# medical-genomics-group/VAMPomi

Hardware: AMD Instinct MI355X
Metric: VAMP iterations/s (+ achieved HBM GB/s of the A/A^T kernels) (higher is better)
Workload: dtype f64

## Files before the change

include/vampomi.h:

```cpp
#ifndef VAMPOMI_H
#define VAMPOMI_H

#include <stdint.h>

#ifdef __cplusplus
extern "C" {
#endif

#define VAMPOMI_ABI_VERSION 3
#define VAMPOMI_MAX_L 64
#define VAMPOMI_UNIQUE_ID_BYTES 128

typedef enum {
    VAMPOMI_OK = 0,
    VAMPOMI_ERR_ARG = 1,
    VAMPOMI_ERR_HIP = 2,
    VAMPOMI_ERR_RCCL = 3,
    VAMPOMI_ERR_IO = 4,
    VAMPOMI_ERR_NAN_PHEN = 5,
    VAMPOMI_ERR_STATE = 6,
    VAMPOMI_ERR_OOM = 7,
    VAMPOMI_ERR_MODEL = 8
} vampomi_status;

// ... 95 lines not shown
    int64_t a_passes_ref;
    int64_t a_passes_exec;
    double* prior_hist;
} vampomi_result;

void vampomi_params_default(vampomi_params* p);
vampomi_status vampomi_infere(vampomi_ctx* ctx, const vampomi_params* p, vampomi_result* r);
vampomi_status vampomi_vamp_begin(vampomi_ctx* ctx, const vampomi_params* p, vampomi_result* r);
vampomi_status vampomi_vamp_step(vampomi_ctx* ctx, int* stopped);
vampomi_status vampomi_vamp_end(vampomi_ctx* ctx);
vampomi_status vampomi_step_phases(vampomi_ctx* ctx, double* solve_s, double* step_s);

vampomi_status vampomi_assoc_loo(vampomi_ctx* ctx, const double* est, double* pvals, double* stats,
                                 int mem);
vampomi_status vampomi_assoc_se(vampomi_ctx* ctx, const double* r1, double gam1, double* pvals, int mem);

vampomi_status vampomi_test_metrics(vampomi_ctx* ctx, const double* est, double* r2, double* corr2, int mem);

typedef struct {
    int64_t launches;
    double ms_total;
    double bytes_total;
    double flops_total;
    int64_t timed;
    double ms_timed;
} vampomi_kernel_stat;

typedef struct {
    vampomi_kernel_stat ax;
    vampomi_kernel_stat atx;
    vampomi_kernel_stat ax_k[4];
    vampomi_kernel_stat atx_k[4];
    int64_t a_passes_exec;
    int64_t host_syncs;
    vampomi_kernel_stat loo;
    vampomi_kernel_stat op;
    vampomi_kernel_stat op_k[4];
    vampomi_kernel_stat coll;
} vampomi_stats;

vampomi_status vampomi_set_timing(vampomi_ctx* ctx, int on);
vampomi_status vampomi_get_stats(vampomi_ctx* ctx, vampomi_stats* out);
vampomi_status vampomi_reset_stats(vampomi_ctx* ctx);

vampomi_status vampomi_dev_set_variant(vampomi_ctx* ctx, int which, int variant);
vampomi_status vampomi_dev_prestep_counts(const vampomi_ctx* ctx, int64_t* made, int64_t* used);
vampomi_status vampomi_dev_time_pass(vampomi_ctx* ctx, int which, int K, int reps, double* avg_ms);
vampomi_status vampomi_dev_read_ceiling(vampomi_ctx* ctx, int reps, double* us_med, double* bytes, int* variant);
vampomi_status vampomi_dev_kernel_name(const vampomi_ctx* ctx, int which, int K, int mode, char* out, int cap);
vampomi_status vampomi_dev_ax_plan(int64_t N, int64_t M, int cus, int variant, int K, int* T, int* TR, int* S,
                                   int* grid, int* nslots, char* name, int cap);
vampomi_status vampomi_dev_op_plan(int64_t N, int64_t M, int cus, int variant, int K, int* T, int* S, int* TR,
                                   int* grid, int64_t* nslots, char* name, int cap);
vampomi_status vampomi_dev_op_lds(int64_t N, int64_t M, int cus, int variant, int K, int64_t* out);
vampomi_status vampomi_dev_op_timestamps(vampomi_ctx* ctx, unsigned long long* out, int cap, int* n);
vampomi_status vampomi_dev_mem_plan(int64_t N, int64_t Mt, int nranks, int rank, int cus, int probit, int writer,
                                    int64_t* bytes);
vampomi_status vampomi_dev_op_apply(vampomi_ctx* ctx, int K, const double* ar, const double* qo, const double* p,
                                    const double* z, const double* beta, double diag, double tau, double gam2,
                                    double* d, double* ad, double* dp);

#ifdef __cplusplus
}
#endif
#endif
```

vampomi_amd/_lib.py:

```python
from __future__ import annotations

import ctypes as C
import os

try:
    import torch
except Exception:
    torch = None

HERE = os.path.dirname(os.path.abspath(__file__))
LIB_PATH = os.environ.get("VAMPOMI_LIB") or os.path.join(HERE, "lib", "libvampomi.so")
CLI_PATH = os.path.join(HERE, "bin", "main_meth.exe")

MAX_L = 64
UNIQUE_ID_BYTES = 128
MEM_HOST, MEM_DEVICE = 0, 1
GEN_GAUSS, GEN_METH = 0, 1

STATUS = {
    0: "OK", 1: "ERR_ARG", 2: "ERR_HIP", 3: "ERR_RCCL", 4: "ERR_IO",
    5: "ERR_NAN_PHEN", 6: "ERR_STATE", 7: "ERR_OOM", 8: "ERR_MODEL",
}


# ... 60 lines not shown
    "vampomi_last_error": (C.c_char_p, []),
    "vampomi_divide_work": (None, [C.c_int64, C.c_int, C.c_int, C.POINTER(C.c_int64), C.POINTER(C.c_int64),
                                   C.POINTER(C.c_int64)]),
    "vampomi_comm_unique_id": (C.c_int, [_P]),
    "vampomi_open": (C.c_int, [C.POINTER(ShardDesc), C.POINTER(_P)]),
    "vampomi_close": (None, [_P]),
    "vampomi_shard_info": (C.c_int, [_P, C.POINTER(C.c_int64), C.POINTER(C.c_int64), C.POINTER(C.c_int64)]),
    "vampomi_sync": (C.c_int, [_P]),
    "vampomi_barrier": (C.c_int, [_P]),
    "vampomi_barrier_timeout": (C.c_int, [_P, C.c_double]),
    "vampomi_load_meth_file": (C.c_int, [_P, C.c_char_p]),
    "vampomi_load_meth_host": (C.c_int, [_P, _P, C.c_int64]),
    "vampomi_generate_meth": (C.c_int, [_P, C.c_uint64, C.c_int]),
    "vampomi_read_phen": (C.c_int, [_P, C.c_char_p, C.c_int]),
    "vampomi_set_phen": (C.c_int, [_P, _P, C.c_int]),
    "vampomi_get_phen": (C.c_int, [_P, _P]),
    "vampomi_simulate_phen": (C.c_int, [_P, C.c_uint64, C.c_double, C.c_double, _P]),
    "vampomi_simulate_phen_binary": (C.c_int, [_P, C.c_uint64, C.c_double, C.c_double, _P]),
    "vampomi_get_marker_stats": (C.c_int, [_P, _P, _P]),
    "vampomi_read_markers": (C.c_int, [_P, C.c_int64, C.c_int64, _P]),
    "vampomi_ax": (C.c_int, [_P, _P, _P, C.c_int]),
    "vampomi_atx": (C.c_int, [_P, _P, _P, C.c_int]),
    "vampomi_lmmse_mult": (C.c_int, [_P, _P, C.c_double, C.c_double, _P, C.c_int]),
    "vampomi_pcg": (C.c_int, [_P, _P, _P, C.c_double, C.c_double, C.c_int, C.c_int, C.c_double, _P,
                              C.POINTER(C.c_int), C.c_int]),
    "vampomi_test_metrics": (C.c_int, [_P, _P, C.POINTER(C.c_double), C.POINTER(C.c_double), C.c_int]),
    "vampomi_assoc_loo": (C.c_int, [_P, _P, _P, _P, C.c_int]),
    "vampomi_assoc_se": (C.c_int, [_P, _P, C.c_double, _P, C.c_int]),
    "vampomi_update_prior": (C.c_int, [_P, _P, C.c_double, C.POINTER(C.c_int), _P, _P, C.c_int, C.c_double,
                                        C.c_int, C.c_double, C.c_int]),
    "vampomi_denoise_bin": (C.c_int, [_P, _P, C.c_double, _P, C.POINTER(C.c_double), C.c_int]),
    "vampomi_denoise": (C.c_int, [_P, _P, C.c_double, _P, _P, C.c_int, _P, _P, C.POINTER(C.c_double), C.c_int]),
    "vampomi_params_default": (None, [C.POINTER(Params)]),
    "vampomi_infere": (C.c_int, [_P, C.POINTER(Params), C.POINTER(Result)]),
    "vampomi_vamp_begin": (C.c_int, [_P, C.POINTER(Params), C.POINTER(Result)]),
    "vampomi_vamp_step": (C.c_int, [_P, C.POINTER(C.c_int)]),
    "vampomi_step_phases": (C.c_int, [_P, C.POINTER(C.c_double), C.POINTER(C.c_double)]),
    "vampomi_vamp_end": (C.c_int, [_P]),
    "vampomi_set_timing": (C.c_int, [_P, C.c_int]),
    "vampomi_get_stats": (C.c_int, [_P, C.POINTER(Stats)]),
    "vampomi_reset_stats": (C.c_int, [_P]),
    "vampomi_dev_set_variant": (C.c_int, [_P, C.c_int, C.c_int]),
    "vampomi_dev_prestep_counts": (C.c_int, [_P, C.POINTER(C.c_int64), C.POINTER(C.c_int64)]),
    "vampomi_dev_time_pass": (C.c_int, [_P, C.c_int, C.c_int, C.c_int, C.POINTER(C.c_double)]),
    "vampomi_dev_read_ceiling": (C.c_int, [_P, C.c_int, C.POINTER(C.c_double), C.POINTER(C.c_double),
                                           C.POINTER(C.c_int)]),
    "vampomi_dev_kernel_name": (C.c_int, [_P, C.c_int, C.c_int, C.c_int, C.c_char_p, C.c_int]),
    "vampomi_dev_mem_plan": (C.c_int, [C.c_int64, C.c_int64, C.c_int, C.c_int, C.c_int, C.c_int, C.c_int, _P]),
    "vampomi_dev_ax_plan": (C.c_int, [C.c_int64, C.c_int64, C.c_int, C.c_int, C.c_int, _P, _P, _P, _P, _P, C.c_char_p,
                                      C.c_int]),
    "vampomi_dev_op_plan": (C.c_int, [C.c_int64, C.c_int64, C.c_int, C.c_int, C.c_int, _P, _P, _P, _P, _P, C.c_char_p,
                                      C.c_int]),
    "vampomi_dev_op_lds": (C.c_int, [C.c_int64, C.c_int64, C.c_int, C.c_int, C.c_int, _P]),
    "vampomi_dev_op_apply": (C.c_int, [_P, C.c_int, _P, _P, _P, _P, _P, C.c_double, C.c_double, C.c_double, _P, _P,
                                       _P]),
    "vampomi_dev_op_timestamps": (C.c_int, [_P, _P, C.c_int, C.POINTER(C.c_int)]),
    "vampomi_all_ok": (C.c_int, [_P, C.c_int, C.POINTER(C.c_int)]),
    "vampomi_comm_abort": (C.c_int, [_P]),
}

_lib = None


def load() -> C.CDLL:
    global _lib
    if _lib is None:
        if not os.path.exists(LIB_PATH):
            raise ImportError(f"{LIB_PATH} not built: run `python -m vampomi_amd.build`")
        lib = C.CDLL(LIB_PATH, mode=C.RTLD_GLOBAL)
        other = bool(os.environ.get("VAMPOMI_LIB"))
        for name, (res, args) in SIGNATURES.items():
            if other and not hasattr(lib, name):
                continue
            f = getattr(lib, name)
            f.restype = res
            f.argtypes = args
        _lib = lib
    return _lib


def check(status: int) -> None:
    if status != 0:
        msg = load().vampomi_last_error()
        raise VampomiError(status, msg.decode() if msg else "")
```

vampomi_amd/csrc/atax_team.hip:

```cpp
#include <hip/hip_ext.h>

#include <algorithm>
#include <cstdio>
#include <mutex>
#include <string>

#include "kdev.h"

namespace vk {

typedef unsigned int v4u __attribute__((ext_vector_type(4)));
typedef unsigned int v2u __attribute__((ext_vector_type(2)));

#ifndef TM_FMA
#define TM_FMA 1
#endif
#ifndef TM_SAFE
#define TM_SAFE 0
#endif
#ifndef TM_TS
#define TM_TS 0
#endif
#ifndef TM_TEAMS_BY_XCD
#define TM_TEAMS_BY_XCD 1
// ... 145 lines not shown
    const double* p[K];
    double* d[K];
    double* sraw[K];
    double diag[K], tau[K], gam2[K];
};
template <int K>
__device__ __forceinline__ TmSlots<K> tm_slots(const OpArgs& a, int alt) {
    TmSlots<K> s;
#pragma unroll
    for (int k = 0; k < K; ++k) {
        int idx = k == alt ? kOpMaxK : k;
        asm volatile("" : "+s"(idx));
        const OpAlt::Slot& t = a.alt.tab[idx];
        s.ar[k] = t.ar;
        s.p[k] = t.p;
        s.d[k] = t.d;
        s.sraw[k] = t.sraw;
        s.diag[k] = t.diag;
        s.tau[k] = t.tau;
        s.gam2[k] = t.gam2;
    }
    return s;
}

template <int K, int S, int F, int L, int P, bool COMM, int E, bool FMA, int KP>
__device__ __forceinline__ void atax_team_body(const double* __restrict__ X, int64_t ld, int64_t N, int64_t M,
                                               const double* __restrict__ mave, const double* __restrict__ msig,
                                               const OpArgs& a, int T, int TR, int ilv,
                                               const int* __restrict__ gate) {
    extern __shared__ __attribute__((aligned(16))) double lds[];
    double* s_beta = lds;
    if (a.fold.on) {
        double& s_go = lds[kOpMaxK];
        if (threadIdx.x == 0) {
            CgState cs = *a.fold.src;
            double r[3 * kMaxRhs];
#pragma unroll
            for (int q = 0; q < 3 * kMaxRhs; ++q) r[q] = q < 3 * cs.K ? a.fold.red[q] : 0.0;
            const bool ran = cg_decide_into(cs, r, a.fold.it, a.fold.mask);
            if (blockIdx.x == 0) {
                *a.fold.dst = cs;
                cg_publish(cs, ran, a.fold.it, a.fold.mirror, a.fold.flag, a.fold.seq, a.fold.pack);
            }
            s_go = cs.any ? 1.0 : 0.0;
#pragma unroll
            for (int k = 0; k < kOpMaxK; ++k) s_beta[k] = cs.beta[k];
        }
        __syncthreads();
        if (s_go == 0.0) return;
    } else if (gate && !*gate) {
        return;
    }
    const double* beta = a.fold.on ? s_beta : a.beta;
    static_assert(K + KP <= kMaxRhs, "partial slots per team");
    int fuse = a.fuse, alt = -1;
    if constexpr (KP == 0) {
        if (a.alt.cs && !a.fold.on) alt = cg_pre_slot(a.alt.cs->active, K, *a.alt.done == a.alt.token);
        if (alt >= 0) fuse &= ~(1 << alt);
    }
#if TM_TS
    const unsigned long long ts0 = __builtin_amdgcn_s_memrealtime();
#endif
    const int dbg = TM_ABL ? TM_ABL : (TM_DBG || !COMM) ? a.dbg : 0;
    constexpr int CW = COMM ? 7 : 8;
    constexpr int RS = tm_rows_per_step(COMM, E);
    static_assert(E == 1 || E == 2, "doubles per lane per load");
    constexpr int RING = F + L + 1;
    static_assert(COMM || L == 0, "without a hand-off the column is finished in its own step");
    static_assert(!COMM || (P >= 1 && P <= L), "polls in flight");
    static_assert(!COMM || P < RING, "a poll's slot is consumed before it is reissued");
    const int wave = threadIdx.x >> 6, lane = threadIdx.x & 63;
    const int g = blockIdx.x >> 3;
    const int member = g % T;
    const int nteams = gridDim.x / T;
#if TM_TEAMS_BY_XCD
    const int team = g / T + (nteams >> 3) * (int)(blockIdx.x & 7);
#else
    const int team = (blockIdx.x & 7) + 8 * (g / T);
#endif
    const int64_t cs = ilv ? nteams : 1;
    const int64_t mb = ilv ? team : (int64_t)team * M / nteams;
    const int n = (int)(ilv ? (M - team + nteams - 1) / nteams : (int64_t)(team + 1) * M / nteams - mb);
    const int64_t nmax = (M + nteams - 1) / nteams;
    const int64_t gwords = (M + gridDim.x) * kOpMaxK * T * 2;
    const int64_t r0 = (int64_t)member * TR;
    const int nrows = (int)(N - r0 < TR ? N - r0 : TR);
    constexpr bool QFULL = tm_qfull(K, S, COMM, E);
    const TmLds lay = tm_lds(K, S, COMM, E, TR < N ? TR : N);
    const int QS = (int)lay.qs;
    double* q_lds = lds + lay.q;
    double* s_part = lds + lay.part;
    double* s_tot = lds + lay.tot;
    const int jb = 64 * E * wave + E * lane;
    const int nbytes = (E == 2 ? (nrows + 1) & ~1 : nrows) * 8;

    if (COMM && wave == CW) {
        const TmSlots<K> sl = tm_slots<K>(a, alt);
        const int nq = K * T;
        unsigned long long* xg = a.xg + (int64_t)team * nmax * nq * 2;
        unsigned long long* dummy = a.xg + gwords + (int64_t)blockIdx.x * 2 * K;
        const bool qv = (lane >> 5) < K && (lane & 31) < T;
        const int ql2 = qv ? 2 * ((lane >> 5) * T + (lane & 31)) : 0;
        const int nq2 = 2 * nq;
        const int csi = (int)cs;
        const unsigned tag = a.tag;
        const double* scp = msig;
#pragma unroll
        for (int k = 0; k < K; ++k) {
            if (lane == 1 + k) scp = sl.p[k];
            if (lane == 1 + K + k && ((fuse >> k) & 1)) scp = a.z.p[k];
        }
// ... 301 lines not shown
                    if (threadIdx.x == 0) {
                        if (a.sraw.p[0]) sl.sraw[k][mg] = t;
                        sl.d[k][mg] = val;
                    }
                    dpacc[k] += val * p;
                }
                cc[k] = sg * val;
            }
        }
#pragma unroll
        for (int s = 0; s < S; ++s) {
            if (dbg & 8) break;
#pragma unroll
            for (int k = 0; k < K; ++k)
#pragma unroll
                for (int e = 0; e < E; ++e) {
                    if constexpr (FMA)
                        acc[k][s][e] = __builtin_fma(xr[slot][s][e], cc[k], acc[k][s][e]);
                    else
                        acc[k][s][e] += xr[slot][s][e] * cc[k];
                }
        }
    };
    if (n > 0) {
        for (int base = -F;; base += RING) {
            if (base - L >= n) break;
#pragma unroll
            for (int i = 0; i < RING; ++i) {
                const int m = base + i;
                load((i + F) % RING, m + F < n ? m + F : n - 1);
                if (m >= 0 && m < n) dot(i, m & 1);
                __syncthreads();
                const int cf = m - L;
                if (cf >= 0 && cf < n) {
                    double tot[K];
                    if (COMM) {
#pragma unroll
                        for (int k = 0; k < K; ++k) tot[k] = s_tot[(cf & 1) * K + k];
                    } else {
#pragma unroll
                        for (int k = 0; k < K; ++k) {
                            double t = 0.0;
#pragma unroll
                            for (int w = 0; w < CW; ++w) t += s_part[((m & 1) * CW + w) * K + k];
                            tot[k] = t;
                        }
                    }
                    finish((i + RING - L) % RING, cf, tot);
                }
            }
        }
    }
    double* dst = a.part + (int64_t)team * kMaxRhs * ld + r0;
#pragma unroll
    for (int s = 0; s < S; ++s) {
        const int jl = RS * s + jb;
        if (jl >= nrows) continue;
#pragma unroll
        for (int k = 0; k < K; ++k)
#pragma unroll
            for (int e = 0; e < E; ++e)
                if (jl + e < nrows) dst[(int64_t)k * ld + jl + e] = acc[k][s][e];
        if constexpr (KP > 0) {
#pragma unroll
            for (int k = 0; k < KP; ++k)
#pragma unroll
                for (int e = 0; e < E; ++e)
                    if (jl + e < nrows) dst[(int64_t)(K + k) * ld + jl + e] = accp[k][s][e];
        }
    }
    if constexpr (COMM) {
        __syncthreads();
    } else if (threadIdx.x == 0) {
#pragma unroll
        for (int k = 0; k < K; ++k) red_put(a.ro, (int64_t)blockIdx.x * K + k, dpacc[k]);
    }
    if (wave == 0) ticket_sum_blocks<K>(a.ro);
#if TM_TS
    if (a.ts && threadIdx.x == 0) {
        unsigned xcc, hw;
        asm volatile("s_getreg_b32 %0, hwreg(HW_REG_XCC_ID)" : "=s"(xcc));
        asm volatile("s_getreg_b32 %0, hwreg(HW_REG_HW_ID)" : "=s"(hw));
        unsigned long long* t = a.ts + 4 * (int64_t)blockIdx.x;
        t[0] = ts0;
        t[1] = __builtin_amdgcn_s_memrealtime();
        t[2] = xcc;
        t[3] = hw;
    }
#endif
}

template <int K, int S, int F, int L, int P, bool COMM, int E, bool FMA>
__global__ __launch_bounds__(kTmThreads) void atax_team_kernel(const double* __restrict__ X, int64_t ld, int64_t N,
                                                               int64_t M, const double* __restrict__ mave,
                                                               const double* __restrict__ msig, OpArgs a, int T,
                                                               int TR, int ilv, const int* __restrict__ gate) {
    atax_team_body<K, S, F, L, P, COMM, E, FMA, 0>(X, ld, N, M, mave, msig, a, T, TR, ilv, gate);
}

static constexpr int kTmPlain = kOpPlain;
template <int S, int F, int L, int P, bool COMM, int E, bool FMA>
__global__ __launch_bounds__(kTmThreads) void atax_team_plain_kernel(const double* __restrict__ X, int64_t ld,
                                                                     int64_t N, int64_t M,
                                                                     const double* __restrict__ mave,
                                                                     const double* __restrict__ msig, OpArgs a, int T,
                                                                     int TR, int ilv, const int* __restrict__ gate) {
    atax_team_body<1, S, F, L, P, COMM, E, FMA, kTmPlain>(X, ld, N, M, mave, msig, a, T, TR, ilv, gate);
}

#ifndef AX_TEAM_SYNC
#define AX_TEAM_SYNC 1
#endif
#ifndef AX_TEAM_F
#define AX_TEAM_F 4
#endif
static constexpr int kAxTmF = AX_TEAM_F;
static constexpr int kAxTmMaxS = 4;
template <int S, int KP, bool FU>
__global__ __launch_bounds__(kTmThreads) void ax_team_kernel(const double* __restrict__ X, int64_t ld, int64_t N,
                                                             int64_t M, const double* __restrict__ mave,
                                                             const double* __restrict__ msig, CPtrs xs,
                                                             double* __restrict__ part, AxFuse fu, int T, int TR) {
    if (fu.gate && !*fu.gate) return;
    constexpr int E = 2, F = kAxTmF, RING = F + 1;
    constexpr int RS = tm_rows_per_step(false, E);
    const int wave = threadIdx.x >> 6, lane = threadIdx.x & 63;
    const int g = blockIdx.x >> 3;
    const int member = g % T;
    const int nteams = gridDim.x / T;
    const int team = g / T + (nteams >> 3) * (int)(blockIdx.x & 7);
    const int n = team < M ? (int)((M - team + nteams - 1) / nteams) : 0;
    const int64_t r0 = (int64_t)member * TR;
    const int nrows = (int)(N - r0 < TR ? N - r0 : TR);
    const int nbytes = ((nrows + 1) & ~1) * 8;
    const int jb = 64 * E * wave + E * lane;
    double bk[KP];
#pragma unroll
    for (int k = 0; k < KP; ++k) bk[k] = FU ? fu.beta[k] : 0.0;
    const double* pkp = mave;
    if (lane == 1) pkp = msig;
#pragma unroll
    for (int k = 0; k < KP; ++k) {
        if (lane == 2 + k) pkp = xs.p[k];
        if (FU && lane == 2 + KP + k) pkp = fu.z.p[k];
    }
    pkp += team;
    double acc[KP][S][E];
#pragma unroll
    for (int k = 0; k < KP; ++k)
#pragma unroll
        for (int s = 0; s < S; ++s)
#pragma unroll
            for (int e = 0; e < E; ++e) acc[k][s][e] = 0.0;
    double xr[RING][S][E];
    double pk[RING];
    const char* xtile = reinterpret_cast<const char*>(X + (int64_t)team * ld + r0);
    auto load = [&](int slot, int m) {
        const int64_t c = (int64_t)m * nteams;
        pk[slot] = pkp[c];
        const __amdgpu_buffer_rsrc_t rs =
// ... 52 lines not shown
    }
}

static int tm_S(int64_t rows, bool comm, int E) {
    const int rs = tm_rows_per_step(comm, E);
    return (int)((rows + rs - 1) / rs);
}

bool team_plan(int64_t N, int64_t M, int cus, int T, int cfg, OpPlan* out) {
    if (cfg < 0 || cfg >= kTmNCfg || N < 1) return false;
    const TmCfg& c = kTmCfg[cfg];
    if ((T == 1) == c.comm) return false;
    if (T < 1 || T > kTmMaxT || (T & (T - 1))) return false;
    const int grid = (cus / (8 * T)) * 8 * T;
    if (grid < T) return false;
    int64_t TR = N;
    if (T > 1) {
        TR = c.E == 2 ? ((N + T - 1) / T + 127) / 128 * 128 : (N + T - 1) / T;
        if ((int64_t)(T - 1) * TR >= N) return false;
    }
    const int S = tm_S(TR, c.comm, c.E);
    if (S > c.maxS) return false;
    for (int K = 1; K <= kOpMaxK; ++K)
        if (tm_lds(K, S, c.comm, c.E, std::min<int64_t>(TR, N)).words * 8 > kTmLdsMaxBytes) return false;
    OpPlan p{};
    p.grid = grid;
    p.S = S;
    p.T = T;
    p.TR = (int)TR;
    p.cfg = cfg;
    p.nslots = grid / T;
    (void)M;
    *out = p;
    return true;
}

bool team_lds_layout(const OpPlan& pl, int64_t N, int K, int64_t out[6]) {
    if (pl.T < 1 || pl.cfg < 0 || pl.cfg >= kTmNCfg || K < 1 || K > kOpMaxK || N < 1) return false;
    const TmCfg& c = kTmCfg[pl.cfg];
    const TmLds l = tm_lds(K, pl.S, c.comm, c.E, std::min<int64_t>(pl.TR, N));
    out[0] = kTmLdsHead;
    out[1] = l.q;
    out[2] = l.qs;
    out[3] = l.part;
    out[4] = l.tot;
    out[5] = l.words;
    return true;
}

template <int K, int S, int C, bool PL>
static hipError_t launch_tm(const Shard& s, const OpPlan& pl, const OpArgs& a, hipStream_t st, const Timing& tm,
                            const int* gate, int* occ) {
    constexpr TmCfg c = kTmCfg[C];
    static_assert(!PL || K == 1, "the head-start kernel has one operator system");
    void (*kern)(const double*, int64_t, int64_t, int64_t, const double*, const double*, OpArgs, int, int, int,
                 const int*);
    if constexpr (PL)
        kern = atax_team_plain_kernel<S, c.F, c.L, c.P, c.comm, c.E, (bool)TM_FMA>;
    else
        kern = atax_team_kernel<K, S, c.F, c.L, c.P, c.comm, c.E, (bool)TM_FMA>;
    const size_t lds = (size_t)tm_lds(K, S, c.comm, c.E, std::min<int64_t>(pl.TR, s.N)).words * sizeof(double);
    if (lds > (size_t)kTmLdsMaxBytes) return hipErrorInvalidValue;
    static std::atomic<unsigned long long> allowed{0};
    if (const hipError_t e = lds_allow(reinterpret_cast<const void*>(kern), allowed, (int)kTmLdsMaxBytes))
        return e;
    if (occ) {
        if (hipOccupancyMaxActiveBlocksPerMultiprocessor(occ, kern, kTmThreads, lds) != hipSuccess) *occ = 0;
        return hipSuccess;
    }
    hipExtLaunchKernelGGL(kern, dim3(pl.grid), dim3(kTmThreads), lds, st, tm.start, tm.stop, 0, s.X, s.ld, s.N, s.M,
                          s.mave, s.msig, a, pl.T, pl.TR, c.ilv ? 1 : 0, gate);
    return hipSuccess;
}

static constexpr int tm_plain_maxS(int cfg) {
    return cfg == 0 ? 8 : cfg == 2 ? 3 : cfg == 3 ? 4 : cfg == 4 ? 5 : 0;
}

template <int K, int C, int S, bool PL>
static hipError_t launch_tm_if(const Shard& s, const OpPlan& pl, const OpArgs& a, hipStream_t st, const Timing& tm,
                               const int* gate, int* occ) {
    if constexpr (S <= (PL ? tm_plain_maxS(C) : kTmCfg[C].maxS))
        return launch_tm<K, S, C, PL>(s, pl, a, st, tm, gate, occ);
    return hipErrorInvalidValue;
}

template <int K, int C, bool PL>
static hipError_t launch_tm_s(int S, const Shard& s, const OpPlan& pl, const OpArgs& a, hipStream_t st,
                        const Timing& tm, const int* gate, int* occ) {
    switch (S) {
        case 1: return launch_tm_if<K, C, 1, PL>(s, pl, a, st, tm, gate, occ);
        case 2: return launch_tm_if<K, C, 2, PL>(s, pl, a, st, tm, gate, occ);
        case 3: return launch_tm_if<K, C, 3, PL>(s, pl, a, st, tm, gate, occ);
        case 4: return launch_tm_if<K, C, 4, PL>(s, pl, a, st, tm, gate, occ);
        case 5: return launch_tm_if<K, C, 5, PL>(s, pl, a, st, tm, gate, occ);
        case 6: return launch_tm_if<K, C, 6, PL>(s, pl, a, st, tm, gate, occ);
        case 7: return launch_tm_if<K, C, 7, PL>(s, pl, a, st, tm, gate, occ);
        case 8: return launch_tm_if<K, C, 8, PL>(s, pl, a, st, tm, gate, occ);
        case 9: return launch_tm_if<K, C, 9, PL>(s, pl, a, st, tm, gate, occ);
        case 10: return launch_tm_if<K, C, 10, PL>(s, pl, a, st, tm, gate, occ);
        default: return hipErrorInvalidValue;
    }
}

static OpArgs tm_with_slots(const OpArgs& a, int K) {
    OpArgs x = a;
    for (int k = 0; k < K && k < kOpMaxK; ++k)
        x.alt.tab[k] = OpAlt::Slot{a.ar.p[k], a.p.p[k], a.d.p[k], a.sraw.p[k], a.diag, a.tau, a.gam2};
    x.alt.tab[kOpMaxK] = OpAlt::Slot{a.alt.ar, a.alt.p, a.alt.d, a.sraw.p[0] ? a.alt.d : nullptr, 1.0, 1.0, 0.0};
    return x;
}

template <int K, bool PL = false>
static hipError_t launch_tm_c(const Shard& s, const OpPlan& pl, const OpArgs& a0, hipStream_t st, const Timing& tm,
                        const int* gate, int* occ = nullptr) {
    const OpArgs a = tm_with_slots(a0, K);
    if constexpr (PL) {
        switch (pl.cfg) {
            case 0: return launch_tm_s<1, 0, true>(pl.S, s, pl, a, st, tm, gate, occ);
            case 2: return launch_tm_s<1, 2, true>(pl.S, s, pl, a, st, tm, gate, occ);
            case 3: return launch_tm_s<1, 3, true>(pl.S, s, pl, a, st, tm, gate, occ);
            case 4: return launch_tm_s<1, 4, true>(pl.S, s, pl, a, st, tm, gate, occ);
            default: return hipErrorInvalidValue;
        }
    }
    switch (pl.cfg) {
        case 0: return launch_tm_s<K, 0, false>(pl.S, s, pl, a, st, tm, gate, occ);
        case 1: return launch_tm_s<K, 1, false>(pl.S, s, pl, a, st, tm, gate, occ);
        case 2: return launch_tm_s<K, 2, false>(pl.S, s, pl, a, st, tm, gate, occ);
        case 3: return launch_tm_s<K, 3, false>(pl.S, s, pl, a, st, tm, gate, occ);
        case 4: return launch_tm_s<K, 4, false>(pl.S, s, pl, a, st, tm, gate, occ);
        case 5: return launch_tm_s<K, 5, false>(pl.S, s, pl, a, st, tm, gate, occ);
        case 6: return launch_tm_s<K, 6, false>(pl.S, s, pl, a, st, tm, gate, occ);
        default: return hipErrorInvalidValue;
    }
}

hipError_t atax_team(const Shard& s, const OpPlan& pl, int K, const OpArgs& a, hipStream_t st, const Timing& tm,
                     const int* gate) {
    if (pl.T < 1 || pl.grid < pl.T || pl.grid % pl.T) return hipErrorInvalidValue;
    if (pl.T > 1 && (!a.xg || !a.err || a.tag == 0)) return hipErrorInvalidValue;
    if (s.M <= 0) return hipSuccess;
    hipError_t e = hipErrorInvalidValue;
    switch (K) {
        case 1: e = launch_tm_c<1>(s, pl, a, st, tm, gate); break;
        case 2: e = launch_tm_c<2>(s, pl, a, st, tm, gate); break;
        default: break;
    }
    if (e != hipSuccess) return e;
    return hipGetLastError();
}

hipError_t atax_team_plain(const Shard& s, const OpPlan& pl, const OpArgs& a, hipStream_t st, const Timing& tm,
                           const int* gate) {
    if (pl.T < 1 || pl.grid < pl.T || pl.grid % pl.T) return hipErrorInvalidValue;
    if (pl.T > 1 && (!a.xg || !a.err || a.tag == 0)) return hipErrorInvalidValue;
    for (int k = 0; k < kTmPlain; ++k)
        if (!a.px.p[k]) return hipErrorInvalidValue;
    if (s.M <= 0) return hipSuccess;
    if (const hipError_t e = launch_tm_c<1, true>(s, pl, a, st, tm, gate)) return e;
    return hipGetLastError();
}

bool ax_team_plan(int64_t N, int64_t M, int cus, AxPlan* out) {
    if (N < 1 || cus < 8) return false;
    constexpr int RS = tm_rows_per_step(false, 2);
    for (int T = 1; T <= kTmMaxT; T *= 2) {
        if (cus / (8 * T) < 1) break;
        const int grid = (cus / (8 * T)) * 8 * T;
        const int64_t TR = T == 1 ? N : ((N + T - 1) / T + 127) / 128 * 128;
        if ((int64_t)(T - 1) * TR >= N) continue;
        const int S = (int)((TR + RS - 1) / RS);
        if (S > kAxTmMaxS) continue;
        AxPlan p{};
        p.variant = kAxTeam;
        p.T = T;
        p.TR = (int)TR;
        p.S = S;
        p.groups = grid;
        p.nslots = grid / T;
        p.rows = N;
        p.tiles = 1;
        p.total = M;
        p.sa = p.nslots;
        p.sb = 1;
        *out = p;
        return true;
    }
    return false;
}

template <int S, int K, bool FU>
static void launch_axt(const Shard& s, const AxPlan& pl, CPtrs x, double* part, hipStream_t st, const Timing& tm,
                       const AxFuse& fu) {
    hipExtLaunchKernelGGL((ax_team_kernel<S, K, FU>), dim3(pl.groups), dim3(kTmThreads), 0, st, tm.start, tm.stop, 0,
                          s.X, s.ld, s.N, s.M, s.mave, s.msig, x, part, fu, pl.T, pl.TR);
}

template <int S>
static bool launch_axt_k(int K, bool fused, const Shard& s, const AxPlan& pl, CPtrs x, double* part,
                         hipStream_t st, const Timing& tm, const AxFuse& fu) {
    switch (K * 2 + (fused ? 1 : 0)) {
        case 2: launch_axt<S, 1, false>(s, pl, x, part, st, tm, fu); return true;
        case 3: launch_axt<S, 1, true>(s, pl, x, part, st, tm, fu); return true;
        case 4: launch_axt<S, 2, false>(s, pl, x, part, st, tm, fu); return true;
        case 5: launch_axt<S, 2, true>(s, pl, x, part, st, tm, fu); return true;
        case 6: launch_axt<S, 3, false>(s, pl, x, part, st, tm, fu); return true;
        case 7: launch_axt<S, 3, true>(s, pl, x, part, st, tm, fu); return true;
        case 8: launch_axt<S, 4, false>(s, pl, x, part, st, tm, fu); return true;
        case 9: launch_axt<S, 4, true>(s, pl, x, part, st, tm, fu); return true;
        default: return false;
    }
}

hipError_t ax_team(const Shard& s, const AxPlan& pl, int K, CPtrs x, double* part, hipStream_t st, const Timing& tm,
                   const AxFuse& fu) {
    if (pl.T < 1 || pl.groups % (8 * pl.T) || pl.nslots != pl.groups / pl.T || pl.S < 1 || pl.S > kAxTmMaxS ||
        (int64_t)(pl.T - 1) * pl.TR >= s.N || (int64_t)pl.T * pl.TR < s.N ||
        (int64_t)pl.S * tm_rows_per_step(false, 2) < std::min<int64_t>(pl.TR, s.N) || pl.rows < s.N)
        return hipErrorInvalidValue;
    if (s.M <= 0) return hipSuccess;
    const bool fused = fu.z.p[0] != nullptr;
    if (fused && !fu.beta) return hipErrorInvalidValue;
    bool ok = false;
    switch (pl.S) {
        case 1: ok = launch_axt_k<1>(K, fused, s, pl, x, part, st, tm, fu); break;
        case 2: ok = launch_axt_k<2>(K, fused, s, pl, x, part, st, tm, fu); break;
        case 3: ok = launch_axt_k<3>(K, fused, s, pl, x, part, st, tm, fu); break;
        case 4: ok = launch_axt_k<4>(K, fused, s, pl, x, part, st, tm, fu); break;
        default: break;
    }
    if (!ok) return hipErrorInvalidValue;
    return hipGetLastError();
}

std::string ax_kernel_name(int K, bool fused, const AxPlan& pl) {
    if (pl.T <= 0) return kernel_name(0, K, fused ? 1 : 0, pl.variant);
    char b[96];
    std::snprintf(b, sizeof b, "ax_team_kernel<%d, %d, %s>", pl.S, K, fused ? "true" : "false");
    return b;
}

bool team_plain_plan(int64_t N, int64_t M, int cus, const OpPlan& main, OpPlan* out) {
    const int cfgs1[] = {0};
    const int cfgsT[] = {2, 3, 4};
    for (int T = std::max(main.T, 1); T <= kTmMaxT; T *= 2) {
        const int* cf = T == 1 ? cfgs1 : cfgsT;
        const int ncf = T == 1 ? 1 : 3;
        for (int i = 0; i < ncf; ++i) {
            OpPlan p{};
            if (!team_plan(N, M, cus, T, cf[i], &p) || p.S > tm_plain_maxS(cf[i])) continue;
            *out = p;
            return true;
        }
    }
    return false;
}

int team_occupancy(const OpPlan& pl, int K) {
    int occ = 0;
    const Shard s{nullptr, 0, (int64_t)pl.TR * pl.T, 1, nullptr, nullptr};
    const OpArgs a{};
    hipError_t e = hipErrorInvalidValue;
    switch (K) {
        case 1: e = launch_tm_c<1>(s, pl, a, nullptr, Timing{}, nullptr, &occ); break;
        case 2: e = launch_tm_c<2>(s, pl, a, nullptr, Timing{}, nullptr, &occ); break;
        case 1 + kTmPlain: e = launch_tm_c<1, true>(s, pl, a, nullptr, Timing{}, nullptr, &occ); break;
        default: break;
    }
    return e == hipSuccess ? occ : 0;
}

std::string team_kernel_name(int K, const OpPlan& pl) {
    const TmCfg& c = kTmCfg[pl.cfg];
    char b[128];
    if (K == 1 + kTmPlain)
        std::snprintf(b, sizeof b, "atax_team_plain_kernel<%d, %d, %d, %d, %s, %d>", pl.S, c.F, c.L, c.P,
                      c.comm ? "true" : "false", c.E);
    else
        std::snprintf(b, sizeof b, "atax_team_kernel<%d, %d, %d, %d, %d, %s, %d>", K, pl.S, c.F, c.L, c.P,
                      c.comm ? "true" : "false", c.E);
    return b;
}

}
```

vampomi_amd/csrc/ctx.h:

```cpp
#pragma once
#include <hip/hip_runtime.h>
#include <rccl/rccl.h>

#include <cstdint>
#include <initializer_list>
#include <memory>
#include <string>
#include <utility>
#include <vector>

#include "../../include/vampomi.h"
#include "kernels.h"

vampomi_status fail(vampomi_status s, const std::string& msg);

#define HIPCHK(expr)                                                                                  \
    do {                                                                                              \
        hipError_t _e = (expr);                                                                       \
        if (_e != hipSuccess)                                                                         \
            return fail(VAMPOMI_ERR_HIP, std::string(#expr) + ": " + hipGetErrorString(_e));          \
    } while (0)

#define NCCLCHK(expr)                                                                                 \
    do {                                                                                              \
// ... 44 lines not shown
    bool mr_tail_req = true;
    bool cg_fold = true;
    bool dp_separate = false;
    bool team_reg = false;
    hipEvent_t team_ev = nullptr;
    ncclComm_t comm = nullptr;
    bool use_comm = false;
    std::shared_ptr<LoopbackComm> loopback;
    std::shared_ptr<ShmComm> shm;
    uint64_t coll_seq = 0;
    bool aborted = false;

    double* X = nullptr;
    double* mave = nullptr;
    double* msig = nullptr;
    double* y = nullptr;
    std::vector<double> y_host;
    bool have_X = false, have_y = false;

    vk::AxPlan axp{};
    int atx_variant = vk::kAtxDefault, loo_variant = vk::kLooDefault;
    double* ax_part = nullptr;
    double* red_part = nullptr;
    size_t red_cap = 0;
    double* scal = nullptr;
    double* h_scal = nullptr;
    double* d_hscal = nullptr;
    unsigned* ticket = nullptr;
    unsigned long long* h_flag = nullptr;
    unsigned long long* d_flag = nullptr;
    unsigned long long sync_seq = 0;
    vk::CgState* cgs = nullptr;
    vk::CgMirror* h_cgm = nullptr;
    vk::CgMirror* d_cgm = nullptr;
    vk::OpPlan opp{};
    int op_variant = vk::kOpDefault;
    bool op_ready = false;
    bool op_ok_mine = false;
    bool op_ok = false;
    bool op_agreed = false;
    int op_variant_req = vk::kOpDefault;
    int cus = 0;
    double* op_part = nullptr;
    int64_t op_part_slots = 0;
    double* op_nvec = nullptr;
    unsigned long long* op_xg = nullptr;
    size_t op_xg_words = 0;
    unsigned op_tag = 0;
    vk::OpPlan opp_hs{};
    bool hs_ok_mine = false;
    bool hs_ok = false;
    bool hs_on = true;
    bool hs_on_req = true;
    int pre_mode = 2;
    unsigned long long pre_seq = 0;
    int64_t pre_made_n = 0, pre_used_n = 0;
    unsigned long long* op_ts = nullptr;
    double* nbuf = nullptr;
    double* mbuf = nullptr;

    bool timing = false;
    int tperiod = 1;
    int64_t tcount[5][vk::kMaxRhs] = {};
    std::vector<TimedLaunch> pending;
    std::vector<hipEvent_t> ev_pool;
    vampomi_stats stats{};

    std::unique_ptr<VampRun> run;
    std::unique_ptr<IterWriter> writer;

    vk::Shard shard() const { return vk::Shard{X, ld, N, M, mave, msig}; }
    vampomi_ctx();
    ~vampomi_ctx();
};

vampomi_status dev_alloc(double** p, size_t n);
void dev_free(double*& p);
vampomi_status host_sync(vampomi_ctx* c);
vampomi_status wait_flag(vampomi_ctx* c, unsigned long long seq, int word = 0);
vampomi_status sync_stream(vampomi_ctx* c, hipStream_t st);
vampomi_status allreduce_dev(vampomi_ctx* c, double* buf, size_t n, const char* site = __builtin_FUNCTION(),
                             int line = __builtin_LINE());
vampomi_status sum_over_ranks(vampomi_ctx* c, double local, double* total, const char* site = __builtin_FUNCTION(),
                              int line = __builtin_LINE());
void comm_abort(vampomi_ctx* c, const std::string& why);
void resolve_timing(vampomi_ctx* c);
TimedLaunch launch_stat(vampomi_ctx* c, int cls, int K, double bytes, double flops);
void drop_launches(vampomi_ctx* c, size_t pending_mark, const vampomi_stats& before);
void release_ctx_resources(vampomi_ctx* c);

vampomi_status ax_dev(vampomi_ctx* c, int K, const double* const* x, double* outbase,
                      const vk::AxFuse* fu = nullptr, const vk::DotArgs* tail = nullptr);
vampomi_status atx_dev(vampomi_ctx* c, int K, const double* const* u, double* const* out, int mode, double tau,
                       double gam2, const double* const* p, const int* gate = nullptr,
                       const double* const* zf = nullptr, const double* beta = nullptr, bool dp = true,
                       double* const* sraw = nullptr);
vampomi_status lmmse_dev(vampomi_ctx* c, int K, const double* const* v, double* const* d, double tau, double gam2,
                         double* nscratch);

class DotBatch {
   public:
    explicit DotBatch(vampomi_ctx* c) : c_(c) {}
    vampomi_status add(std::initializer_list<vk::DotTerm> terms, int64_t n, bool sync, double* out);
    struct Group {
        std::vector<vk::DotTerm> terms;
        bool sync;
// ... 5 lines not shown
    vampomi_status add_pair(int64_t na, const std::vector<Group>& ga, const vk::G1Chain* chain,
                            const double* chain_of, const std::vector<std::pair<const double*, double*>>& ca,
                            int64_t nb, const std::vector<Group>& gb,
                            const std::vector<std::pair<const double*, double*>>& cb);
    vampomi_status sink(int nq, bool sync, double* out, vk::RedOut* ro);
    vampomi_status flush();
    bool empty() const { return sinks_.empty(); }
    const double* dev_result(const double* out) const;
    vampomi_status reduce_now();
    double* dev_slot(const double* out) const;
    hipStream_t stream() const;

   private:
    vampomi_status build(const std::vector<Group>& groups, const vk::G1Chain* chain, const double* chain_of,
                         const std::vector<std::pair<const double*, double*>>& copies, vk::DotArgs& a,
                         vk::RedOut& ro);
    struct Sink {
        int slot, count;
        double* out;
    };
    vampomi_ctx* c_;
    int nsync_ = 0, nlocal_ = 0;
    int nred_ = 0;
    unsigned long long last_seq_ = 0;
    std::vector<Sink> sinks_;
};

inline vk::DotTerm T(const double* a, const double* b, int op = vk::DOT) { return vk::DotTerm{a, b, op}; }

struct CgSystem {
    const double* v = nullptr;
    double* mu = nullptr;
    bool mu0_nonzero = false;
    const double* atx0 = nullptr;
    double* W = nullptr;
    double* S = nullptr;
    double* AW = nullptr;
    bool onsager = false;
    int iters = 0;
    double *r = nullptr, *z = nullptr, *p = nullptr, *d = nullptr;
};
struct HeadStart {
    double* abern = nullptr;
    const double* xnext = nullptr;
    double* axnext = nullptr;
    bool used = false;
    double* T1 = nullptr;
    double* U1 = nullptr;
    unsigned long long* pre_done = nullptr;
    bool pre_have = false;
    bool pre_offer = false;
    bool pre_made = false;
    bool pre_used = false;
};
enum class PreMode { normal, ahead, queued };
struct PcgArgs {
    double tau = 0.0, gam2 = 0.0;
    int max_iter = 0;
    double tol = 0.0;
    double* nscratch = nullptr;
    int64_t* ref_passes = nullptr;
    DotBatch* init = nullptr;
    const double* extra_x = nullptr;
    double* ex_out = nullptr;
    bool onepass = false;
    const double* const* ar0 = nullptr;
    HeadStart* hs = nullptr;
    const vk::Prelude* pre = nullptr;
    PreMode pm = PreMode::normal;
};
vampomi_status pcg_run(vampomi_ctx* c, const std::vector<CgSystem*>& sys, const PcgArgs& args);
vampomi_status op_prepare(vampomi_ctx* c);
vampomi_status op_agree(vampomi_ctx* c);
vampomi_status headstart_available(vampomi_ctx* c, bool* yes);
constexpr int64_t kPreMinBytes = (int64_t)256 << 20;
bool prestep_on(const vampomi_ctx* c);
unsigned* op_err_dev(vampomi_ctx* c);
vampomi_status op_check_err(vampomi_ctx* c);
vampomi_status op_dev(vampomi_ctx* c, int K, const vk::OpArgs& a, const int* gate, bool reduce = true,
                      bool divide = true);
vampomi_status op_dev_plain(vampomi_ctx* c, const vk::OpArgs& a, const double* const* px, double* const* out,
                            const int* gate);
```

vampomi_amd/csrc/engine.cpp:

```cpp
#include <hip/hip_runtime.h>
#include <rccl/rccl.h>

#include <algorithm>
#include <atomic>
#include <cfloat>
#include <chrono>
#include <condition_variable>
#include <map>
#include <mutex>
#include <cmath>
#include <cstdio>
#include <cstdlib>
#include <cstring>
#include <memory>
#include <string>
#include <thread>
#include <vector>

#include <fcntl.h>
#include <unistd.h>

#include "ctx.h"
#include "hostio.h"
#include "writer.h"
// ... 605 lines not shown
        HIPCHK(vk::ax_reduce(c->axp, K, c->N, c->ld, c->ax_part, os, c->sqrtN, c->st, f.gate));
    } else {
        HIPCHK(vk::ax_reduce(c->axp, K, c->N, c->ld, c->ax_part, os, 0.0, c->st, f.gate));
        size_t n = (size_t)K * c->ld;
        if (tail) {
            HIPCHK(vk::dots(*tail, c->M, vk::RedOut{c->red_part, outbase + n, c->ticket, nullptr, 0, f.gate}, c->st));
            n += (size_t)tail->nt;
        }
        STCHK(allreduce_dev(c, outbase, n));
        HIPCHK(vk::vec_div(K, c->N, c->ld, os, c->sqrtN, c->st));
    }
    return VAMPOMI_OK;
}

vampomi_status atx_dev(vampomi_ctx* c, int K, const double* const* u, double* const* out, int mode,
                              double tau, double gam2, const double* const* p, const int* gate,
                              const double* const* zf, const double* beta, bool dp, double* const* sraw) {
    if (!c->have_X) return fail(VAMPOMI_ERR_STATE, "ATx before the methylation data was loaded");
    if (c->M <= 0) return VAMPOMI_OK;
    vk::CPtrs us{}, ps{}, zs{};
    vk::Ptrs os{}, ss{};
    for (int k = 0; k < K; ++k) {
        us.p[k] = u[k];
        os.p[k] = out[k];
        ss.p[k] = sraw ? sraw[k] : nullptr;
        ps.p[k] = p ? p[k] : nullptr;
        zs.p[k] = zf ? zf[k] : nullptr;
    }
    TimedLaunch t = launch_stat(c, 1, K, pass_bytes(c, K), pass_flops(c, K));
    HIPCHK(vk::atx(c->shard(), K, us, os, 1.0 / c->sqrtN, mode, tau, gam2, ps, c->st, c->atx_variant, vk::Timing{t.a, t.b}, gate, zs,
                   zf ? beta : nullptr, ss));
    c->stats.a_passes_exec++;
    if (mode == 1 && dp) {
        vk::DotArgs a{};
        a.nt = K;
        for (int k = 0; k < K; ++k)
            a.t[k] = zf ? vk::DotTerm{out[k], p[k], vk::PUPD, zf[k], beta + k} : vk::DotTerm{out[k], p[k], vk::DOT};
        HIPCHK(vk::dots(a, c->M, vk::RedOut{c->red_part, c->scal + SL_DP, c->ticket, nullptr, 0, gate}, c->st));
        STCHK(allreduce_dev(c, c->scal + SL_DP, K));
    }
    return VAMPOMI_OK;
}

static size_t red_capacity(int64_t Mx) {
    return std::max<size_t>({(size_t)vk::kRedBlocks * 3 * vk::kMaxRhs, (size_t)vk::kRedBlocks * vk::kMaxTerms,
                             (size_t)((Mx + 255) / 256) * (1 + 2 * (vk::kMaxL - 1)),
                             (size_t)(Mx / 8 + 1) * vk::kMaxRhs, (size_t)4096});
}

static size_t op_xg_words_for(int64_t Mx, const vk::OpPlan& p) {
    return (size_t)(Mx + p.grid) * vk::kOpMaxK * (size_t)p.T * 2 + (size_t)p.grid * (2 * vk::kOpMaxK + 1);
}

static vampomi_status op_plan_local(vampomi_ctx* c) {
    if (c->cus <= 0) HIPCHK(hipDeviceGetAttribute(&c->cus, hipDeviceAttributeMultiprocessorCount, c->device));
    const int64_t M = std::max<int64_t>(c->M, 1);
    bool op_ok = vk::op_plan(c->N, M, c->cus, c->op_variant, &c->opp);
    if (op_ok && c->opp.T >= 1) {
        for (int K = 1; K <= vk::kOpMaxK && op_ok; ++K) {
            const int occ = vk::team_occupancy(c->opp, K);
            if ((int64_t)occ * c->cus < c->opp.grid) {
                std::fprintf(stderr, "libvampomi: one-pass operator off: %s fits %d workgroup(s) per CU; the plan "
                                     "needs %lld resident on %d CUs (two passes per CG step)\n",
                             vk::team_kernel_name(K, c->opp).c_str(), occ, (long long)c->opp.grid, c->cus);
                op_ok = false;
            }
        }
    }
    bool hs_ok = op_ok && vk::team_plain_plan(c->N, M, c->cus, c->opp, &c->opp_hs);
    if (hs_ok && (int64_t)vk::team_occupancy(c->opp_hs, 1 + vk::kOpPlain) * c->cus < c->opp_hs.grid) hs_ok = false;
    c->op_ok_mine = op_ok;
    c->hs_ok_mine = hs_ok;
    if (!c->op_ts && std::getenv("VAMPOMI_OP_TS") && std::atoi(std::getenv("VAMPOMI_OP_TS"))) {
        HIPCHK(hipMalloc((void**)&c->op_ts, (size_t)4 * 8 * std::max(c->cus, 1) * 2));
        HIPCHK(hipMemsetAsync(c->op_ts, 0, (size_t)4 * 8 * std::max(c->cus, 1) * 2, c->st));
    }
    if (!c->op_nvec) {
        STCHK(dev_alloc(&c->op_nvec, (size_t)3 * vk::kMaxRhs * c->ld + 16));
        HIPCHK(hipMemsetAsync(c->op_nvec, 0, ((size_t)3 * vk::kMaxRhs * c->ld + 16) * 8, c->st));
    }
    if (op_ok) {
        const int64_t slots = std::max<int64_t>(c->opp.nslots, hs_ok ? c->opp_hs.nslots : 0);
        if (slots > c->op_part_slots) {
            dev_free(c->op_part);
            STCHK(dev_alloc(&c->op_part, (size_t)slots * vk::kMaxRhs * c->ld));
            c->op_part_slots = slots;
        }
        if (c->opp.T > 1 || (hs_ok && c->opp_hs.T > 1)) {
            size_t words = c->opp.T > 1 ? op_xg_words_for(M, c->opp) : 0;
            if (hs_ok && c->opp_hs.T > 1) words = std::max(words, op_xg_words_for(M, c->opp_hs));
            if (words > c->op_xg_words) {
                if (c->op_xg) (void)hipFree(c->op_xg);
                c->op_xg = nullptr;
                c->op_xg_words = 0;
                HIPCHK(hipMalloc((void**)&c->op_xg, words * 8));
                HIPCHK(hipMemsetAsync(c->op_xg, 0, words * 8, c->st));
                c->op_xg_words = words;
            }
        }
    }
    c->op_ready = true;
    return VAMPOMI_OK;
}

vampomi_status op_prepare(vampomi_ctx* c) {
    if (!c->op_ready) STCHK(op_plan_local(c));
    if (!c->use_comm) {
        c->op_ok = c->op_ok_mine;
        c->hs_ok = c->hs_ok_mine && c->hs_on;
    } else if (!c->op_agreed) {
        c->op_ok = c->hs_ok = false;
    }
    return VAMPOMI_OK;
}

vampomi_status op_agree(vampomi_ctx* c) {
    if (!c->use_comm) return VAMPOMI_OK;
    if (c->op_variant_req != c->op_variant || c->hs_on_req != c->hs_on) {
        c->op_variant = c->op_variant_req;
        c->hs_on = c->hs_on_req;
        c->op_ready = false;
    }
    bool op = false, hs = false;
    if (c->have_X) {
        if (!c->op_ready) STCHK(op_plan_local(c));
        op = c->op_ok_mine;
        hs = c->hs_ok_mine;
    }
    const double mine = (op ? 0.0 : 1.0) + (hs ? 0.0 : 1024.0) + (c->hs_on ? 0.0 : 1048576.0) +
                        (c->mr_tail_req ? 0.0 : 1073741824.0);
    double all = 0.0;
    STCHK(sum_over_ranks(c, mine, &all));
    const int64_t a = (int64_t)all;
    c->op_ok = a % 1024 == 0;
    c->hs_ok = c->op_ok && (a / 1024) % 1024 == 0 && (a / 1048576) % 1024 == 0;
    c->mr_tail = a / 1073741824 == 0;
    c->op_agreed = true;
    return VAMPOMI_OK;
// ... 63 lines not shown
    HIPCHK(launch());
    if (!g.last) HIPCHK(hipEventCreateWithFlags(&g.last, hipEventDisableTiming));
    HIPCHK(hipEventRecord(g.last, c->st));
    return VAMPOMI_OK;
}

vampomi_status op_check_err(vampomi_ctx* c) {
    const unsigned e = c->h_flag ? __atomic_exchange_n(reinterpret_cast<unsigned*>(c->h_flag + 4), 0u, __ATOMIC_ACQ_REL) : 0u;
    if (e > 1)
        return fail(VAMPOMI_ERR_HIP, "one-pass operator: address checks failed (codes " + std::to_string(e >> 1) + ")");
    if (e)
        return fail(VAMPOMI_ERR_HIP, "one-pass operator: a team hand-off timed out (a workgroup of the team never "
                                     "ran: fewer compute units than planned?)");
    return VAMPOMI_OK;
}

vampomi_status op_dev(vampomi_ctx* c, int K, const vk::OpArgs& a, const int* gate, bool reduce, bool divide) {
    if (!c->have_X) return fail(VAMPOMI_ERR_STATE, "A before the methylation data was loaded");
    STCHK(op_prepare(c));
    if (!c->op_ok || K < 1 || K > vk::kOpMaxK)
        return fail(VAMPOMI_ERR_ARG, "one-pass operator: K <= 2 and a plan for N = " + std::to_string(c->N));
    double* ad = c->op_nvec + (int64_t)2 * vk::kMaxRhs * c->ld;
    vk::OpArgs x = a;
    x.part = c->op_part;
    x.scale = 1.0 / c->sqrtN;
    if (c->opp.T > 1) {
        x.xg = c->op_xg;
        if (++c->op_tag == 0) ++c->op_tag;
        x.tag = c->op_tag;
        x.err = op_err_dev(c);
    }
    static const int dbg = std::getenv("VAMPOMI_OP_DBG") ? std::atoi(std::getenv("VAMPOMI_OP_DBG")) : 0;
    x.dbg = dbg;
    x.ts = c->op_ts;
    x.ro = vk::RedOut{c->red_part, c->use_comm ? ad + (int64_t)K * c->ld : c->scal + SL_DP, c->ticket, nullptr, 0,
                      gate};
    TimedLaunch t = launch_stat(c, 3, K, pass_bytes(c, K), 2.0 * pass_flops(c, K));
    STCHK(team_launch(c, c->opp.T,
                      [&] { return vk::atax(c->shard(), c->opp, K, x, c->st, vk::Timing{t.a, t.b}, gate); }));
    c->stats.a_passes_exec++;
    vk::Ptrs os{};
    for (int k = 0; k < K; ++k) os.p[k] = ad + (int64_t)k * c->ld;
    if (!c->use_comm) {
        if (reduce) HIPCHK(vk::op_reduce(c->opp, K, c->N, c->ld, c->op_part, os, c->sqrtN, c->st, gate));
    } else {
        HIPCHK(vk::op_reduce(c->opp, K, c->N, c->ld, c->op_part, os, 0.0, c->st, gate));
        STCHK(allreduce_dev(c, ad, (size_t)K * c->ld + K));
        if (divide) HIPCHK(vk::vec_div(K, c->N, c->ld, os, c->sqrtN, c->st));
    }
    return VAMPOMI_OK;
}

vampomi_status op_dev_plain(vampomi_ctx* c, const vk::OpArgs& a, const double* const* px, double* const* out,
                            const int* gate) {
    if (!c->have_X) return fail(VAMPOMI_ERR_STATE, "A before the methylation data was loaded");
    STCHK(op_prepare(c));
    if (!c->hs_ok) return fail(VAMPOMI_ERR_ARG, "head-start launch: no plan for N = " + std::to_string(c->N));
    constexpr int KT = 1 + vk::kOpPlain;
    double* ad = c->op_nvec + (int64_t)2 * vk::kMaxRhs * c->ld;
    vk::OpArgs x = a;
    x.part = c->op_part;
    x.scale = 1.0 / c->sqrtN;
    for (int k = 0; k < vk::kOpPlain; ++k) x.px.p[k] = px[k];
    if (c->opp_hs.T > 1) {
        x.xg = c->op_xg;
        if (++c->op_tag == 0) ++c->op_tag;
        x.tag = c->op_tag;
        x.err = op_err_dev(c);
    }
    x.dbg = 0;
    x.ro = vk::RedOut{c->red_part, c->use_comm ? ad + (int64_t)KT * c->ld : c->scal + SL_DP, c->ticket, nullptr, 0,
                      gate};
    TimedLaunch t = launch_stat(c, 3, KT, pass_bytes(c, KT), pass_flops(c, 1) + pass_flops(c, KT));
    STCHK(team_launch(c, c->opp_hs.T, [&] {
        return vk::atax_team_plain(c->shard(), c->opp_hs, x, c->st, vk::Timing{t.a, t.b}, gate);
    }));
    c->stats.a_passes_exec++;
    if (!c->use_comm) {
        vk::Ptrs os{};
        for (int k = 0; k < vk::kOpPlain; ++k) os.p[k] = out[k];
        HIPCHK(vk::op_reduce(c->opp_hs, vk::kOpPlain, c->N, c->ld, c->op_part, os, c->sqrtN, c->st, gate, 1));
    } else {
        vk::Ptrs os{};
        for (int k = 0; k < KT; ++k) os.p[k] = ad + (int64_t)k * c->ld;
        HIPCHK(vk::op_reduce(c->opp_hs, KT, c->N, c->ld, c->op_part, os, 0.0, c->st, gate));
        STCHK(allreduce_dev(c, ad, (size_t)KT * c->ld + 1));
        vk::Ptrs dst = os;
        for (int k = 0; k < vk::kOpPlain; ++k) dst.p[1 + k] = out[k];
        HIPCHK(vk::vec_div(KT, c->N, c->ld, os, c->sqrtN, c->st, &dst));
    }
    return VAMPOMI_OK;
}

vampomi_status lmmse_dev(vampomi_ctx* c, int K, const double* const* v, double* const* d, double tau,
                                double gam2, double* nscratch) {
    STCHK(ax_dev(c, K, v, nscratch));
    const double* u[vk::kMaxRhs];
    for (int k = 0; k < K; ++k) u[k] = nscratch + (int64_t)k * c->ld;
    return atx_dev(c, K, u, d, 1, tau, gam2, v);
}

extern "C" int vampomi_abi_version(void) { return VAMPOMI_ABI_VERSION; }
extern "C" const char* vampomi_last_error(void) { return g_err.c_str(); }

extern "C" void vampomi_divide_work(int64_t Mt, int nranks, int rank, int64_t* M, int64_t* S, int64_t* Mm) {
    const int64_t modu = Mt % nranks, size = Mt / nranks;
    int64_t cum = 0;
    for (int r = 0; r < nranks; ++r) {
        const int64_t len = r < modu ? size + 1 : size;
        if (r == rank) {
            if (M) *M = len;
            if (S) *S = cum;
        }
        cum += len;
    }
    if (Mm) *Mm = modu != 0 ? size + 1 : size;
}

extern "C" vampomi_status vampomi_comm_unique_id(void* out) {
    if (!out) return fail(VAMPOMI_ERR_ARG, "null argument");
    ncclUniqueId id;
    NCCLCHK(ncclGetUniqueId(&id));
    static_assert(sizeof(ncclUniqueId) == VAMPOMI_UNIQUE_ID_BYTES, "unique id size");
    std::memcpy(out, &id, sizeof id);
    return VAMPOMI_OK;
}

void release_ctx_resources(vampomi_ctx* c) {
    (void)hipSetDevice(c->device);
    if (c->st) (void)hipStreamSynchronize(c->st);
    team_gate_leave(c);
    resolve_timing(c);
    for (auto e : c->ev_pool) (void)hipEventDestroy(e);
    c->ev_pool.clear();
// ... 41 lines not shown
    if (d->Mt < d->nranks) return fail(VAMPOMI_ERR_ARG, "every rank needs at least one marker (Mt >= nranks)");
    std::unique_ptr<vampomi_ctx> c(new vampomi_ctx());
    c->rank = d->rank;
    c->nranks = d->nranks;
    c->N = d->N;
    c->Mt = d->Mt;
    c->alpha_scale = d->alpha_scale == 0.0 ? 1.0 : d->alpha_scale;
    vampomi_divide_work(c->Mt, c->nranks, c->rank, &c->M, &c->S, &c->Mm);
    c->ld = (c->N + 15) / 16 * 16;
    c->sqrtN = std::sqrt((double)c->N);
    int ndev = 0;
    HIPCHK(hipGetDeviceCount(&ndev));
    if (ndev < 1) return fail(VAMPOMI_ERR_HIP, "no HIP device visible");
    c->device = d->device >= 0 ? d->device : c->rank % ndev;
    HIPCHK(hipSetDevice(c->device));
    HIPCHK(hipStreamCreateWithFlags(&c->st, hipStreamNonBlocking));
    team_gate_join(c.get());
    const int64_t Mx = std::max<int64_t>(c->M, 1);
    c->axp = vk::ax_plan(c->N, Mx);
    STCHK(dev_alloc(&c->mave, Mx));
    STCHK(dev_alloc(&c->msig, Mx));
    STCHK(dev_alloc(&c->y, c->ld));
    HIPCHK(hipMemsetAsync(c->y, 0, c->ld * 8, c->st));
    STCHK(dev_alloc(&c->ax_part, (size_t)c->axp.nslots * vk::kMaxRhs * c->ld));
    c->red_cap = red_capacity(Mx);
    STCHK(dev_alloc(&c->red_part, c->red_cap));
    c->writer.reset(new IterWriter());
    STCHK(c->writer->open(c.get()));
    STCHK(dev_alloc(&c->scal, SL_TOTAL));
    HIPCHK(hipHostMalloc((void**)&c->h_scal, SL_TOTAL * sizeof(double), hipHostMallocMapped | hipHostMallocCoherent));
    HIPCHK(hipHostGetDevicePointer((void**)&c->d_hscal, c->h_scal, 0));
    HIPCHK(hipHostMalloc((void**)&c->h_flag, 64, hipHostMallocMapped | hipHostMallocCoherent));
    std::memset(c->h_flag, 0, 64);
    HIPCHK(hipHostGetDevicePointer((void**)&c->d_flag, c->h_flag, 0));
    HIPCHK(hipMalloc((void**)&c->ticket, 64 * sizeof(unsigned)));
    HIPCHK(hipMemsetAsync(c->ticket, 0, 64 * sizeof(unsigned), c->st));
    STCHK(dev_alloc(&c->nbuf, (size_t)vk::kMaxRhs * c->ld));
    HIPCHK(hipMemsetAsync(c->nbuf, 0, (size_t)vk::kMaxRhs * c->ld * 8, c->st));
    STCHK(dev_alloc(&c->mbuf, (size_t)2 * vk::kMaxRhs * Mx));
    HIPCHK(hipMalloc((void**)&c->cgs, 2 * sizeof(vk::CgState)));
    HIPCHK(hipMemsetAsync(c->cgs, 0, 2 * sizeof(vk::CgState), c->st));
    HIPCHK(hipHostMalloc((void**)&c->h_cgm, vk::kCgMirrorSlots * sizeof(vk::CgMirror),
                         hipHostMallocMapped | hipHostMallocCoherent));
    std::memset(c->h_cgm, 0, vk::kCgMirrorSlots * sizeof(vk::CgMirror));
    HIPCHK(hipHostGetDevicePointer((void**)&c->d_cgm, c->h_cgm, 0));
    const char* force = std::getenv("VAMPOMI_FORCE_RCCL");
    c->use_comm = c->nranks > 1 || (force && std::atoi(force) != 0);
    if (const char* mv = std::getenv("VAMPOMI_MR_TAIL")) c->mr_tail = c->mr_tail_req = std::atoi(mv) != 0;
    if (const char* fv = std::getenv("VAMPOMI_CG_FOLD")) c->cg_fold = std::atoi(fv) != 0;
    if (const char* dv = std::getenv("VAMPOMI_DP_SEPARATE")) c->dp_separate = std::atoi(dv) != 0;
    if (const char* hv = std::getenv("VAMPOMI_HEADSTART")) c->hs_on = c->hs_on_req = std::atoi(hv) != 0;
    if (const char* pv = std::getenv("VAMPOMI_PRESTEP")) {
        const int v = std::atoi(pv);
        if (v >= 0 && v <= 2) c->pre_mode = v;
    }
    const char* mode = std::getenv("VAMPOMI_COMM");
    if (c->use_comm && mode && std::strcmp(mode, "loopback") == 0) {
        if (!d->comm_id) return fail(VAMPOMI_ERR_ARG, "the loopback communicator needs a communicator id");
        c->loopback = loopback_join(d->comm_id, c->nranks);
    } else if (c->use_comm && mode && std::strcmp(mode, "shm") == 0) {
        if (!d->comm_id) return fail(VAMPOMI_ERR_ARG, "the shm communicator needs a communicator id");
        std::string err;
        c->shm = shm_join(d->comm_id, c->nranks, c->rank, comm_init_timeout_s(), &err);
        if (!c->shm) return fail(VAMPOMI_ERR_STATE, err);
    } else if (c->use_comm) {
        ncclUniqueId id;
        if (d->comm_id)
            std::memcpy(&id, d->comm_id, sizeof id);
        else
            NCCLCHK(ncclGetUniqueId(&id));
        ncclConfig_t cfg = NCCL_CONFIG_INITIALIZER;
        cfg.blocking = 0;
        STCHK(nccl_settle(c.get(), ncclCommInitRankConfig(&c->comm, c->nranks, id, c->rank, &cfg),
                          "ncclCommInitRankConfig", comm_init_timeout_s()));
    }
    STCHK(sync_stream(c.get(), c->st));
    *out = c.release();
    return VAMPOMI_OK;
}

extern "C" vampomi_status vampomi_shard_info(const vampomi_ctx* c, int64_t* M, int64_t* S, int64_t* ld) {
    if (!c) return fail(VAMPOMI_ERR_ARG, "null context");
    if (M) *M = c->M;
    if (S) *S = c->S;
    if (ld) *ld = c->ld;
    return VAMPOMI_OK;
}

extern "C" vampomi_status vampomi_sync(vampomi_ctx* c) {
    if (!c) return fail(VAMPOMI_ERR_ARG, "null context");
    HIPCHK(hipSetDevice(c->device));
    STCHK(sync_stream(c, c->st));
    return VAMPOMI_OK;
}

extern "C" vampomi_status vampomi_barrier(vampomi_ctx* c) {
    CollScope cs_(c);
    if (!c) return fail(VAMPOMI_ERR_ARG, "null context");
    if (c->use_comm) STCHK(allreduce_dev(c, c->scal + SL_BARRIER, 1));
    STCHK(sync_stream(c, c->st));
    return VAMPOMI_OK;
}

extern "C" vampomi_status vampomi_barrier_timeout(vampomi_ctx* c, double seconds) {
    if (!c || !(seconds > 0)) return fail(VAMPOMI_ERR_ARG, "null context or no limit");
    c->coll_limit_s = seconds;
    const vampomi_status st = vampomi_barrier(c);
// ... 460 lines not shown
    for (auto pr : {std::make_pair(&out->ax, out->ax_k), std::make_pair(&out->atx, out->atx_k),
                    std::make_pair(&out->op, out->op_k)}) {
        int64_t n = 0;
        double ms = 0.0;
        for (int k = 0; k < 4; ++k) {
            n += pr.second[k].launches;
            ms += pr.second[k].ms_total;
        }
        if (n == pr.first->launches) pr.first->ms_total = ms;
        else fill(*pr.first);
    }
    return VAMPOMI_OK;
}

extern "C" vampomi_status vampomi_reset_stats(vampomi_ctx* c) {
    if (!c) return fail(VAMPOMI_ERR_ARG, "null context");
    STCHK(sync_stream(c, c->st));
    resolve_timing(c);
    c->stats = vampomi_stats{};
    return VAMPOMI_OK;
}

extern "C" vampomi_status vampomi_dev_set_variant(vampomi_ctx* c, int which, int variant) {
    if (!c) return fail(VAMPOMI_ERR_ARG, "null context");
    HIPCHK(hipSetDevice(c->device));
    STCHK(sync_stream(c, c->st));
    if (which == 0) {
        if (!vk::ax_variant_ok(variant)) return fail(VAMPOMI_ERR_ARG, "no such A.x variant");
        const vk::AxPlan np = vk::ax_plan(c->N, std::max<int64_t>(c->M, 1), variant);
        if (np.nslots > c->axp.nslots) {
            dev_free(c->ax_part);
            STCHK(dev_alloc(&c->ax_part, (size_t)np.nslots * vk::kMaxRhs * c->ld));
        }
        c->axp = np;
    } else if (which == 1) {
        if (!vk::atx_variant_ok(variant)) return fail(VAMPOMI_ERR_ARG, "no such A^T.u variant");
        c->atx_variant = variant;
    } else if (which == 3) {
        vk::OpPlan p{};
        if (!vk::op_plan(c->N, std::max<int64_t>(c->M, 1), c->cus > 0 ? c->cus : 256, variant, &p))
            return fail(VAMPOMI_ERR_ARG, "no such one-pass operator plan for this N");
        c->op_variant_req = variant;
        if (!c->use_comm) {
            c->op_variant = variant;
            c->op_ready = false;
        }
    } else if (which == 4) {
        return fail(VAMPOMI_ERR_ARG, "no side stream: every launch runs on the context's stream (DESIGN.md §6)");
    } else if (which == 5) {
        if (variant != 0 && variant != 1) return fail(VAMPOMI_ERR_ARG, "head start: 0 or 1");
        c->hs_on_req = variant == 1;
        if (!c->use_comm) c->hs_on = c->hs_on_req;
    } else if (which == 7) {
        if (variant < 0 || variant > 2) return fail(VAMPOMI_ERR_ARG, "pre-step: 0, 1 or 2");
        c->pre_mode = variant;
    } else if (which == 6) {
        if (variant != 0 && variant != 1) return fail(VAMPOMI_ERR_ARG, "multi-rank tail: 0 or 1");
        c->mr_tail_req = variant == 1;
        if (!c->use_comm) c->mr_tail = c->mr_tail_req;
    } else {
        if (!vk::loo_variant_ok(variant)) return fail(VAMPOMI_ERR_ARG, "no such association-pass variant");
        c->loo_variant = variant;
    }
    return VAMPOMI_OK;
}

bool prestep_on(const vampomi_ctx* c) {
    if (c->use_comm || c->nranks != 1 || !c->hs_ok || c->pre_mode == 0) return false;
    return c->pre_mode == 1 || std::max<int64_t>(c->M, 1) * c->ld * 8 >= kPreMinBytes;
}

extern "C" vampomi_status vampomi_dev_prestep_counts(const vampomi_ctx* c, int64_t* made, int64_t* used) {
    if (!c || !made || !used) return fail(VAMPOMI_ERR_ARG, "null argument");
    *made = c->pre_made_n;
    *used = c->pre_used_n;
    return VAMPOMI_OK;
}

extern "C" vampomi_status vampomi_dev_time_pass(vampomi_ctx* c, int which, int K, int reps, double* avg_ms) {
    if (!c || !avg_ms || K < 1 || K > (which == 0 ? 4 : which == 1 ? 3 : which == 3 ? 2 : 1) || reps < 1)
        return fail(VAMPOMI_ERR_ARG, "bad argument");
    if (!c->have_X) return fail(VAMPOMI_ERR_STATE, "no methylation data loaded");
    HIPCHK(hipSetDevice(c->device));
    if (which == 3) {
        STCHK(op_prepare(c));
        if (!c->op_ok_mine) return fail(VAMPOMI_ERR_ARG, "no one-pass operator plan for this N");
    }
    const int64_t Mx = std::max<int64_t>(c->M, 1);
    vk::CPtrs in{};
    vk::Ptrs out{};
    for (int k = 0; k < K; ++k) {
        in.p[k] = which == 0 ? c->mbuf + k * Mx : c->nbuf + k * c->ld;
        out.p[k] = which == 0 ? c->nbuf + k * c->ld : c->mbuf + k * Mx;
    }
    hipEvent_t a, b;
    HIPCHK(hipEventCreate(&a));
    HIPCHK(hipEventCreate(&b));
    HIPCHK(hipEventRecord(a, c->st));
    for (int r = 0; r < reps; ++r) {
        if (which == 0)
            HIPCHK(vk::ax_partial(c->shard(), c->axp, K, in, c->ax_part, c->st));
        else if (which == 1)
            HIPCHK(vk::atx(c->shard(), K, in, out, 1.0 / c->sqrtN, 0, 0.0, 0.0, vk::CPtrs{}, c->st, c->atx_variant));
        else if (which == 3) {
            vk::OpArgs x{};
            for (int k = 0; k < K; ++k) {
                x.ar.p[k] = c->nbuf + k * c->ld;
                x.p.p[k] = c->mbuf + k * Mx;
                x.d.p[k] = c->mbuf + (2 + k) * Mx;
            }
            x.diag = 1.0;
            x.scale = 1.0 / c->sqrtN;
            x.tau = 1.0;
            x.part = c->op_part;
            x.ro = vk::RedOut{c->red_part, c->scal + SL_DP, c->ticket, nullptr, 0, nullptr};
            if (c->opp.T > 1) {
                x.xg = c->op_xg;
                if (++c->op_tag == 0) ++c->op_tag;
                x.tag = c->op_tag;
                x.err = op_err_dev(c);
            }
            x.dbg = std::getenv("VAMPOMI_OP_DBG") ? std::atoi(std::getenv("VAMPOMI_OP_DBG")) : 0;
// ... 54 lines not shown
        a.fuse = (1 << K) - 1;
    }
    a.diag = diag;
    a.tau = tau;
    a.gam2 = gam2;
    STCHK(op_dev(c, K, a, nullptr));
    const double* AD = c->op_nvec + (int64_t)2 * vk::kMaxRhs * c->ld;
    for (int k = 0; k < K; ++k) {
        STCHK(stage_out(c, c->mbuf + (2 + k) * Mx, c->M, VAMPOMI_MEM_HOST, d + k * c->M));
        STCHK(stage_out(c, AD + k * c->ld, c->N, VAMPOMI_MEM_HOST, ad + k * c->N));
    }
    HIPCHK(hipMemcpyAsync(dp, c->scal + SL_DP, (size_t)K * 8, hipMemcpyDeviceToHost, c->st));
    STCHK(sync_stream(c, c->st));
    return op_check_err(c);
}

extern "C" vampomi_status vampomi_dev_op_timestamps(vampomi_ctx* c, unsigned long long* out, int cap, int* n) {
    if (!c || !out || !n) return fail(VAMPOMI_ERR_ARG, "null argument");
    if (!c->op_ts) return fail(VAMPOMI_ERR_STATE, "no timestamps (VAMPOMI_OP_TS=1 at the first operator use)");
    STCHK(sync_stream(c, c->st));
    *n = std::min(cap, 4 * c->opp.grid);
    HIPCHK(hipMemcpy(out, c->op_ts, (size_t)*n * 8, hipMemcpyDeviceToHost));
    return VAMPOMI_OK;
}

extern "C" vampomi_status vampomi_dev_ax_plan(int64_t N, int64_t M, int cus, int variant, int K, int* T, int* TR,
                                              int* S, int* grid, int* nslots, char* name, int cap) {
    if (N < 1 || M < 1 || cus < 1 || K < 1 || K > vk::kMaxRhs || !vk::ax_variant_ok(variant))
        return fail(VAMPOMI_ERR_ARG, "bad argument");
    const vk::AxPlan p = vk::ax_plan_for(N, M, cus, variant);
    if (T) *T = p.T;
    if (TR) *TR = p.TR;
    if (S) *S = p.S;
    if (grid) *grid = p.groups;
    if (nslots) *nslots = p.nslots;
    if (name && cap > 0) std::snprintf(name, (size_t)cap, "%s", vk::ax_kernel_name(K, false, p).c_str());
    return VAMPOMI_OK;
}

extern "C" vampomi_status vampomi_dev_op_plan(int64_t N, int64_t M, int cus, int variant, int K, int* T, int* S,
                                              int* TR, int* grid, int64_t* nslots, char* name, int cap) {
    vk::OpPlan p{};
    if (K < 1 || K > vk::kOpMaxK || !vk::op_plan(N, std::max<int64_t>(M, 1), cus, variant, &p))
        return fail(VAMPOMI_ERR_ARG, "no one-pass operator plan");
    if (T) *T = p.T;
    if (S) *S = p.S;
    if (TR) *TR = p.TR;
    if (grid) *grid = p.grid;
    if (nslots) *nslots = p.nslots;
    if (name && cap > 0) std::snprintf(name, (size_t)cap, "%s", vk::op_kernel_name(K, p).c_str());
    return VAMPOMI_OK;
}

extern "C" vampomi_status vampomi_dev_op_lds(int64_t N, int64_t M, int cus, int variant, int K, int64_t* out) {
    vk::OpPlan p{};
    if (!out || !vk::op_plan(N, std::max<int64_t>(M, 1), cus, variant, &p) || !vk::team_lds_layout(p, N, K, out))
        return fail(VAMPOMI_ERR_ARG, "no team plan with that system count");
    return VAMPOMI_OK;
}

extern "C" vampomi_status vampomi_dev_mem_plan(int64_t N, int64_t Mt, int nranks, int rank, int cus, int probit,
                                               int writer, int64_t* bytes) {
    if (!bytes || N < 2 || Mt < nranks || nranks < 1 || rank < 0 || rank >= nranks || cus < 1)
        return fail(VAMPOMI_ERR_ARG, "bad argument");
    int64_t M = 0, S = 0, Mm = 0;
    vampomi_divide_work(Mt, nranks, rank, &M, &S, &Mm);
    const int64_t Mx = std::max<int64_t>(M, 1), ld = (N + 15) / 16 * 16;
    int64_t total = 0;
    auto add = [&](int64_t n, int64_t elem) {
        const int64_t b = std::max<int64_t>(n, 1) * elem, g = 2 << 20;
        total += (b + g - 1) / g * g;
    };
    const vk::AxPlan axp = vk::ax_plan(N, Mx);
    add(Mx * ld, 8);
    add(Mx, 8), add(Mx, 8), add(ld, 8);
    add((int64_t)axp.nslots * vk::kMaxRhs * ld, 8);
    add((int64_t)red_capacity(Mx), 8), add((int64_t)red_capacity(Mx), 8);
    add(SL_TOTAL, 8), add(64, 4), add(64, 4);
    add((int64_t)vk::kMaxRhs * ld, 8);
    add((int64_t)2 * vk::kMaxRhs * Mx, 8);
    add((int64_t)sizeof(vk::CgState), 1);
    vk::OpPlan op{}, hs{};
    if (vk::op_plan(N, Mx, cus, vk::kOpDefault, &op)) {
        const bool h = vk::team_plain_plan(N, Mx, cus, op, &hs);
        add((int64_t)3 * vk::kMaxRhs * ld + 16, 8);
        add(std::max<int64_t>(op.nslots, h ? hs.nslots : 0) * vk::kMaxRhs * ld, 8);
        size_t w = op.T > 1 ? op_xg_words_for(Mx, op) : 0;
        if (h && hs.T > 1) w = std::max(w, op_xg_words_for(Mx, hs));
        if (w) add((int64_t)w, 8);
    }
    for (int q = 0; q < 25; ++q) add(Mx, 8);
    add(ld, 8), add((int64_t)vk::kMaxRhs * ld, 8), add((int64_t)vk::kMaxRhs * ld, 8), add(ld, 8);
    add(2 * ld, 8);
    add(Mx, 8), add(ld + 2, 8);
    if (probit) {
        for (int q = 0; q < 3; ++q) add(ld, 8);
        for (int q = 0; q < 3; ++q) add(Mx, 8);
    }
    (void)writer;
    *bytes = total;
    return VAMPOMI_OK;
}

static std::string op_name(const vampomi_ctx* c, int K) {
    vk::OpPlan p{};
    int cus = c->cus;
    if (cus <= 0 && hipDeviceGetAttribute(&cus, hipDeviceAttributeMultiprocessorCount, c->device) != hipSuccess) cus = 256;
    if (!vk::op_plan(c->N, std::max<int64_t>(c->M, 1), cus, c->op_variant, &p)) return "(no one-pass plan)";
    if (K == 1 + vk::kOpPlain) {
        vk::OpPlan h{};
        if (!vk::team_plain_plan(c->N, std::max<int64_t>(c->M, 1), cus, p, &h)) return "(no head-start plan)";
        return vk::team_kernel_name(K, h);
    }
    return vk::op_kernel_name(K, p);
}

extern "C" vampomi_status vampomi_dev_read_ceiling(vampomi_ctx* c, int reps, double* us_med, double* bytes,
                                                   int* variant) {
    if (!c || reps < 1 || !us_med) return fail(VAMPOMI_ERR_ARG, "bad argument");
    if (!c->have_X) return fail(VAMPOMI_ERR_STATE, "no methylation data loaded");
    HIPCHK(hipSetDevice(c->device));
    if (c->cus <= 0) HIPCHK(hipDeviceGetAttribute(&c->cus, hipDeviceAttributeMultiprocessorCount, c->device));
    STCHK(sync_stream(c, c->st));
    const int64_t n = std::max<int64_t>(c->M, 1) * c->ld;
    hipEvent_t a, b;
    HIPCHK(hipEventCreate(&a));
    HIPCHK(hipEventCreate(&b));
    double best = -1.0, best_bytes = 0.0;
    int best_kind = -1;
    for (int kind = 0; kind < 2; ++kind) {
        double nb = 0.0;
        if (vk::stream_read(c->X, n, kind, c->cus, c->st, vk::Timing{}, c->red_part, &nb) != hipSuccess) {
            (void)hipGetLastError();
            continue;
        }
        std::vector<float> ms((size_t)reps);
        for (int r = 0; r < reps; ++r) {
            HIPCHK(vk::stream_read(c->X, n, kind, c->cus, c->st, vk::Timing{a, b}, c->red_part, &nb));
            HIPCHK(hipEventSynchronize(b));
            HIPCHK(hipEventElapsedTime(&ms[(size_t)r], a, b));
        }
        std::sort(ms.begin(), ms.end());
        const double med = 1e3 * (double)ms[(size_t)reps / 2];
        if (best < 0.0 || nb / med > best_bytes / best) {
            best = med;
            best_bytes = nb;
            best_kind = kind;
        }
    }
    (void)hipEventDestroy(a);
    (void)hipEventDestroy(b);
    if (best_kind < 0) return fail(VAMPOMI_ERR_ARG, "the matrix is too small for a read-ceiling stream");
    *us_med = best;
    if (bytes) *bytes = best_bytes;
    if (variant) *variant = best_kind;
    return VAMPOMI_OK;
}

extern "C" vampomi_status vampomi_dev_kernel_name(const vampomi_ctx* c, int which, int K, int mode, char* out,
                                                  int cap) {
    if (!c || !out || cap < 1) return fail(VAMPOMI_ERR_ARG, "bad argument");
    const std::string n = which == 2   ? vk::loo_kernel_name(c->loo_variant)
                          : which == 3 ? op_name(c, K)
                          : which == 0 ? vk::ax_kernel_name(K, mode == 1, c->axp)
                                       : vk::kernel_name(1, K, mode, c->atx_variant);
// ... 4 lines not shown
```

vampomi_amd/csrc/kernels.h:

```cpp
#pragma once
#include <hip/hip_runtime.h>

#include <atomic>
#include <cstdint>
#include <string>

namespace vk {

constexpr int kMaxRhs = 4;
constexpr int kMaxL = 64;
constexpr int kMaxTerms = 12;
constexpr int kRedBlocks = 1024;

struct CPtrs { const double* p[kMaxRhs]; };
struct Timing { hipEvent_t start = nullptr, stop = nullptr; };
struct RedOut {
    double* part;
    double* out;
    unsigned* ticket;
    unsigned long long* flag = nullptr;
    unsigned long long seq = 0;
    const int* gate = nullptr;
    double* out2 = nullptr;
    int split = 0;
// ... 70 lines not shown
struct CgMirror;
struct OpFold {
    const CgState* src = nullptr;
    CgState* dst = nullptr;
    const double* red = nullptr;
    int on = 0, it = 0, mask = 0xf, pack = 0;
    CgMirror* mirror = nullptr;
    unsigned long long* flag = nullptr;
    unsigned long long seq = 0;
};
struct OpAlt {
    const CgState* cs = nullptr;
    const unsigned long long* done = nullptr;
    unsigned long long token = 0;
    const double* ar = nullptr;
    const double* p = nullptr;
    double* d = nullptr;
    struct Slot {
        const double* ar;
        const double* p;
        double* d;
        double* sraw;
        double diag, tau, gam2;
    };
    Slot tab[2 + 1];
};
struct OpArgs {
    CPtrs ar, qo;
    CPtrs p, z;
    const double* beta;
    int fuse;
    double diag, scale, tau, gam2;
    Ptrs d, sraw;
    CPtrs px;
    double* part;
    RedOut ro;
    unsigned long long* xg;
    unsigned tag;
    unsigned* err;
    unsigned long long* ts;
    int dbg;
    OpFold fold;
    OpAlt alt;
};
static_assert(sizeof(OpAlt::tab) / sizeof(OpAlt::Slot) == kOpMaxK + 1, "one entry per system and the alternate's");
std::string op_kernel_name(int K, const OpPlan& pl);
std::string team_kernel_name(int K, const OpPlan& pl);
int team_occupancy(const OpPlan& pl, int K);
hipError_t atax(const Shard& s, const OpPlan& pl, int K, const OpArgs& a, hipStream_t st, const Timing& tm = Timing{},
                const int* gate = nullptr);
hipError_t atax_team(const Shard& s, const OpPlan& pl, int K, const OpArgs& a, hipStream_t st, const Timing& tm,
                     const int* gate);
hipError_t atax_team_plain(const Shard& s, const OpPlan& pl, const OpArgs& a, hipStream_t st, const Timing& tm,
                           const int* gate);
bool team_plain_plan(int64_t N, int64_t M, int cus, const OpPlan& main, OpPlan* out);
hipError_t op_reduce(const OpPlan& pl, int K, int64_t N, int64_t ld, const double* part, Ptrs out, double div,
                     hipStream_t st, const int* gate = nullptr, int k0 = 0);

hipError_t marker_stats(const double* X, int64_t ld, int64_t N, int64_t M, double nonas,
                        double alpha_scale, double* mave, double* msig, hipStream_t st);

hipError_t gen_markers(uint64_t seed, int kind, int64_t N, int64_t ld, int64_t S, int64_t M, double* X,
                       hipStream_t st);
hipError_t gen_beta(uint64_t seed, double lam, int64_t S, int64_t M, double* beta, const RedOut& ro, hipStream_t st);
hipError_t scale_vec(int64_t n, double* v, double a, hipStream_t st);
hipError_t add_noise(uint64_t seed, int64_t N, double sd, double* y, hipStream_t st);

enum DotOp { DOT = 0, DIFF2 = 1, SUM = 2, PUPD = 3, SQPUPD = 4 };
struct DotTerm {
    const double* a;
    const double* b;
    int op;
    const double* c = nullptr;
    const double* beta = nullptr;
};
struct G1Chain {
    int term = 0;
    double gam2 = 0.0, rho = 0.0, gam1_prev = 0.0;
    double* out = nullptr;
};
struct DotCopy {
    int n = 0;
    int term[2] = {0, 0};
    double* dst[2] = {nullptr, nullptr};
};
struct DotArgs {
    DotTerm t[kMaxTerms];
    int nt;
    G1Chain g1;
    DotCopy copy;
};
int red_blocks(int64_t n);
hipError_t dots(const DotArgs& a, int64_t n, const RedOut& ro, hipStream_t st);
hipError_t dots2(const DotArgs& a, int64_t na, const RedOut& roa, const DotArgs& b, int64_t nb, const RedOut& rob,
                 hipStream_t st);

struct Mix {
    double probs[kMaxL];
    double vars[kMaxL];
    int L;
};
constexpr int kMixWords = 2 + 2 * kMaxL;
struct PreOut;
hipError_t denoise(int64_t M, const double* r1, double gam1, const Mix& mix, double* x1,
                   const double* x1_prev, int damp, double rho, double* x1d, const RedOut& ro, hipStream_t st,
                   const double* mixw = nullptr, const double* gam1dev = nullptr, const PreOut* po = nullptr);

struct EmUpd {
    int64_t Mt = 0;
    int learn_vars = 0;
// ... 9 lines not shown
    int L;
    const double* lx;
    const double* ly;
    double la, lb, lc;
    double* r1out;
    const double* dsc;
    EmUpd upd;
};
hipError_t em_sums(int64_t M, const double* r1, const EmArgs& a, const RedOut& ro, hipStream_t st);

hipError_t lincomb_div(int64_t n, double a, const double* x, double b, const double* y, double c,
                       double* out, hipStream_t st);
hipError_t axpby(int64_t n, double a, const double* x, double b, const double* y, double* out,
                 hipStream_t st);
hipError_t bernoulli(uint64_t seed, int it, int64_t S, int64_t M, double sqrtMt, double* out,
                     hipStream_t st);
struct PreOut {
    const double* tn = nullptr;
    const double* tc = nullptr;
    double Mt = 0.0, N = 0.0;
    double* out = nullptr;
    double* mirror = nullptr;
};
struct TailPost {
    int mode = 0;
    const double* src = nullptr;
    G1Chain g1;
    const double* cp_src[2] = {nullptr, nullptr};
    double* cp_dst[2] = {nullptr, nullptr};
    int L = 0;
    double vars[kMaxL] = {};
    EmUpd upd;
    PreOut po;
    const double* gam1dev = nullptr;
};
hipError_t tail_post(const TailPost& t, hipStream_t st);
struct PreDev {
    const double* scal = nullptr;
};
struct Prelude {
    double eta1, gam1, gam2, gamw;
    PreDev dev;
    const double* x1;
    const double* r1;
    const double* atxy;
    double* r2;
    double* v;
    uint64_t seed;
    int it;
    int64_t S;
    double sqrtMt;
    double* bern;
    double* bern_next;
    double* zero[2];
};
hipError_t prelude(int64_t M, const Prelude& p, hipStream_t st);
hipError_t div_scalar(int64_t n, const double* x, double d, double* out, hipStream_t st);
hipError_t div2_scalar(int64_t n, const double* x, const double* r, double d, double* out, hipStream_t st);

hipError_t probit_denoise(int64_t N, const double* p1, const double* y, double tau1, double* z1, const RedOut& ro,
                          hipStream_t st);
hipError_t probit_confusion(int64_t N, int nz, const double* z, int64_t ld, const double* y, const RedOut& ro,
                            hipStream_t st);
hipError_t probit_p1(uint64_t seed, int64_t N, double* p1, hipStream_t st);

hipError_t loo_sums(const Shard& s, const double* ymod, const double* x1, double sqrtN, double* stats,
                    hipStream_t st, int variant = kLooDefault, const Timing& tm = Timing{});
std::string loo_kernel_name(int variant);
int loo_variant_count();
bool loo_variant_ok(int v);
hipError_t loo_pvals(int64_t M, const double* stats, int n, double* pvals, hipStream_t st);
hipError_t se_pvals(int64_t M, const double* r1, double gam1, int64_t N, double* pvals, hipStream_t st);
hipError_t set_scalar(double* p, double v, hipStream_t st);
hipError_t mul_scalar(int64_t n, const double* x, double a, double* out, hipStream_t st);

hipError_t signal_host(unsigned long long* flag, unsigned long long seq, hipStream_t st);
hipError_t post_flag(unsigned long long* flag, unsigned long long seq, hipStream_t st);
hipError_t publish_host(const double* a, int na, double* ha, const double* b, int nb, double* hb,
                        unsigned long long* flag, unsigned long long seq, hipStream_t st);

struct CgVecs {
    double* mu[kMaxRhs];
    double* r[kMaxRhs];
    double* z[kMaxRhs];
    double* p[kMaxRhs];
    const double* d[kMaxRhs];
    const double* v[kMaxRhs];
    const double* atx0[kMaxRhs];
    double tau, gam2;
    double* W[kMaxRhs];
    const double* S[kMaxRhs];
    double* AW[kMaxRhs];
    const double* AS[kMaxRhs];
    int64_t nA;
    double* Q[kMaxRhs];
    double* AR[kMaxRhs];
    const double* AD[kMaxRhs];
    const double* adpart;
    int64_t adld;
    int adslots;
    double addiv;
    double* pre_u1;
    unsigned long long* pre_done;
    unsigned long long pre_token;
};
__host__ __device__ inline int cg_pre_slot(const int* active, int K, bool made) {
// ... 55 lines not shown
```

vampomi_amd/csrc/kernels.hip:

```cpp
#include "kernels.h"
#include "kdev.h"

#include <algorithm>
#include <cstdlib>

#include <hip/hip_ext.h>

#include <hip/hip_runtime.h>

#include <cstdio>
#include <mutex>
#include <string>

namespace vk {

static constexpr int kBlock = 256;

__device__ __forceinline__ double block_sum(double v, double* lds4) {
    v = wave_sum(v);
    const int lane = threadIdx.x & 63, w = threadIdx.x >> 6;
    __syncthreads();
    if (lane == 0) lds4[w] = v;
    __syncthreads();
    return ((lds4[0] + lds4[1]) + lds4[2]) + lds4[3];
// ... 958 lines not shown
        case 10: return launch_op<K, 10>(s, pl, a, st, tm, gate);
        default: return hipErrorInvalidValue;
    }
}

hipError_t atax(const Shard& s, const OpPlan& pl, int K, const OpArgs& a, hipStream_t st, const Timing& tm,
                const int* gate) {
    if (pl.T > 0) return atax_team(s, pl, K, a, st, tm, gate);
    if (K < 1 || K > kOpMaxK || !whole_column_ok(s.N) ||
        pl.S != (int)std::max<int64_t>(1, (s.N + kOpRows - 1) / kOpRows))
        return hipErrorInvalidValue;
    if (s.M <= 0) return hipSuccess;
    hipError_t e = hipErrorInvalidValue;
    switch (K) {
        case 1: e = launch_op_s<1>(pl.S, s, pl, a, st, tm, gate); break;
        case 2: e = launch_op_s<2>(pl.S, s, pl, a, st, tm, gate); break;
        default: break;
    }
    if (e != hipSuccess) return e;
    return hipGetLastError();
}

template <int W = 32>
__device__ __forceinline__ v2d slot_sum(const double* src, int64_t ss, int t0, int t1) {
    v2d acc = {0.0, 0.0};
    int t = t0;
    for (; W >= 32 && t + 32 <= t1; t += 32) {
        v2d x[32];
#pragma unroll
        for (int u = 0; u < 32; ++u) x[u] = *reinterpret_cast<const v2d*>(src + (t + u) * ss);
#pragma unroll
        for (int u = 0; u < 32; ++u) acc += x[u];
    }
    for (; W >= 16 && t + 16 <= t1; t += 16) {
        v2d x[16];
#pragma unroll
        for (int u = 0; u < 16; ++u) x[u] = *reinterpret_cast<const v2d*>(src + (t + u) * ss);
#pragma unroll
        for (int u = 0; u < 16; ++u) acc += x[u];
    }
    for (; t + 8 <= t1; t += 8) {
        v2d x[8];
#pragma unroll
        for (int u = 0; u < 8; ++u) x[u] = *reinterpret_cast<const v2d*>(src + (t + u) * ss);
#pragma unroll
        for (int u = 0; u < 8; ++u) acc += x[u];
    }
    for (; t < t1; ++t) acc += *reinterpret_cast<const v2d*>(src + t * ss);
    return acc;
}

__global__ __launch_bounds__(256) void op_reduce_kernel(int64_t N, int64_t ld, int nslots,
                                                        const double* __restrict__ part, Ptrs out, double div,
                                                        const int* __restrict__ gate) {
    if (gate && !*gate) return;
    __shared__ v2d wsum[4][64];
    const int lane = threadIdx.x & 63, w = threadIdx.x >> 6;
    const int64_t tpk = (N + 127) / 128;
    const int k = (int)(blockIdx.x / tpk);
    const int64_t i = (blockIdx.x - k * tpk) * 128 + 2 * lane;
    const bool ok = i < N;
    wsum[w][lane] = ok ? slot_sum(part + (int64_t)k * ld + i, (int64_t)kMaxRhs * ld, w * nslots / 4,
                                  (w + 1) * nslots / 4)
                       : v2d{0.0, 0.0};
    __syncthreads();
    if (w != 0 || !ok) return;
    v2d r = ((wsum[0][lane] + wsum[1][lane]) + wsum[2][lane]) + wsum[3][lane];
    if (div > 0) r /= div;
    out.p[k][i] = r.x;
    if (i + 1 < N) out.p[k][i + 1] = r.y;
}

hipError_t op_reduce(const OpPlan& pl, int K, int64_t N, int64_t ld, const double* part, Ptrs out, double div,
                     hipStream_t st, const int* gate, int k0) {
    const int64_t n = (int64_t)K * N;
    if (n <= 0) return hipSuccess;
    if (k0 < 0 || k0 + K > kMaxRhs) return hipErrorInvalidValue;
    hipLaunchKernelGGL(op_reduce_kernel, dim3((unsigned)(K * cdiv(N, 128))), dim3(256), 0, st, N, ld, (int)pl.nslots,
                       part + (int64_t)k0 * ld, out, div, gate);
    return hipGetLastError();
}

__global__ __launch_bounds__(kBlock) void stats_kernel(const double* __restrict__ X, int64_t ld, int64_t N, int64_t M,
                                                       double nonas, double alpha_scale, double* __restrict__ mave,
                                                       double* __restrict__ msig) {
    const int lane = threadIdx.x & 63, wave = threadIdx.x >> 6;
    const int64_t m = (int64_t)blockIdx.x * 4 + wave;
    if (m >= M) return;
    const double* col = X + m * ld;
    double s = 0.0;
    for (int64_t j = 2 * lane; j < N; j += 128) {
        const v2d x = ld2(col + j);
        s += x.x;
        if (j + 1 < N) s += x.y;
    }
    s = wave_sum(s);
    const double mean = s / nonas;
    double q = 0.0;
    for (int64_t j = 2 * lane; j < N; j += 128) {
        const v2d x = ld2(col + j);
        const double a = x.x - mean;
        q += a * a;
        if (j + 1 < N) {
            const double b = x.y - mean;
            q += b * b;
        }
    }
    q = wave_sum(q);
    if (lane == 0) {
        mave[m] = mean;
        double sg;
        if (q != 0.0) {
            if (alpha_scale == 1.0)
                sg = 1.0 / sqrt(q / (nonas - 1.0));
            else
                sg = 1.0 / pow(sqrt(q / (nonas - 1.0)), alpha_scale);
        } else {
            sg = 1.0;
        }
        msig[m] = sg;
    }
}

hipError_t marker_stats(const double* X, int64_t ld, int64_t N, int64_t M, double nonas, double alpha_scale,
                        double* mave, double* msig, hipStream_t st) {
    if (M <= 0) return hipSuccess;
    hipLaunchKernelGGL(stats_kernel, dim3((unsigned)cdiv(M, 4)), dim3(kBlock), 0, st, X, ld, N, M, nonas, alpha_scale,
                       mave, msig);
    return hipGetLastError();
}

__global__ void gen_kernel(uint64_t seed, int kind, int64_t N, int64_t ld, int64_t S, int64_t M, double* X) {
// ... 425 lines not shown
}

hipError_t em_sums(int64_t M, const double* r1, const EmArgs& a, const RedOut& ro, hipStream_t st) {
    const int nblk = (int)std::max<int64_t>(1, cdiv(M, kBlock));
    hipLaunchKernelGGL(em_kernel, dim3(nblk), dim3(kBlock), 0, st, M, r1, a, ro);
    return hipGetLastError();
}

__global__ void lincomb_div_kernel(int64_t n, double a, const double* __restrict__ x, double b,
                                   const double* __restrict__ y, double c, double* __restrict__ out) {
    const int64_t i = (int64_t)blockIdx.x * kBlock + threadIdx.x;
    if (i < n) out[i] = (a * x[i] - b * y[i]) / c;
}

hipError_t lincomb_div(int64_t n, double a, const double* x, double b, const double* y, double c, double* out,
                       hipStream_t st) {
    if (n <= 0) return hipSuccess;
    hipLaunchKernelGGL(lincomb_div_kernel, dim3((unsigned)cdiv(n, kBlock)), dim3(kBlock), 0, st, n, a, x, b, y, c,
                       out);
    return hipGetLastError();
}

__global__ void axpby_kernel(int64_t n, double a, const double* __restrict__ x, double b,
                             const double* __restrict__ y, double* __restrict__ out) {
    const int64_t i = (int64_t)blockIdx.x * kBlock + threadIdx.x;
    if (i < n) out[i] = a * x[i] + b * y[i];
}

hipError_t axpby(int64_t n, double a, const double* x, double b, const double* y, double* out, hipStream_t st) {
    if (n <= 0) return hipSuccess;
    hipLaunchKernelGGL(axpby_kernel, dim3((unsigned)cdiv(n, kBlock)), dim3(kBlock), 0, st, n, a, x, b, y, out);
    return hipGetLastError();
}

__global__ void bern_kernel(uint64_t seed, int it, int64_t S, int64_t M, double sqrtMt, double* out) {
    const int64_t i = (int64_t)blockIdx.x * kBlock + threadIdx.x;
    if (i < M) out[i] = (double)(2 * bern_bit(seed, it, S + i) - 1) / sqrtMt;
}

hipError_t bernoulli(uint64_t seed, int it, int64_t S, int64_t M, double sqrtMt, double* out, hipStream_t st) {
    if (M <= 0) return hipSuccess;
    hipLaunchKernelGGL(bern_kernel, dim3((unsigned)cdiv(M, kBlock)), dim3(kBlock), 0, st, seed, it, S, M, sqrtMt,
                       out);
    return hipGetLastError();
}

__global__ void prelude_kernel(int64_t M, Prelude p) {
    const int64_t i = (int64_t)blockIdx.x * kBlock + threadIdx.x;
    if (i >= M) return;
    const double r2 = (p.eta1 * p.x1[i] - p.gam1 * p.r1[i]) / p.gam2;
    p.r2[i] = r2;
    p.v[i] = p.gamw * p.atxy[i] + p.gam2 * r2;
    p.bern[i] = (double)(2 * bern_bit(p.seed, p.it, p.S + i) - 1) / p.sqrtMt;
    if (p.bern_next) p.bern_next[i] = (double)(2 * bern_bit(p.seed, p.it + 1, p.S + i) - 1) / p.sqrtMt;
    if (p.zero[0]) p.zero[0][i] = 0.0;
    if (p.zero[1]) p.zero[1][i] = 0.0;
}

hipError_t prelude(int64_t M, const Prelude& p, hipStream_t st) {
    if (M <= 0) return hipSuccess;
    hipLaunchKernelGGL(prelude_kernel, dim3((unsigned)cdiv(M, kBlock)), dim3(kBlock), 0, st, M, p);
    return hipGetLastError();
}

__global__ void set_scalar_kernel(double* p, double v) {
    if (threadIdx.x == 0) *p = v;
}

hipError_t set_scalar(double* p, double v, hipStream_t st) {
    hipLaunchKernelGGL(set_scalar_kernel, dim3(1), dim3(64), 0, st, p, v);
    return hipGetLastError();
}

__global__ void div_scalar_kernel(int64_t n, const double* __restrict__ x, double d, double* __restrict__ out) {
    const int64_t i = (int64_t)blockIdx.x * kBlock + threadIdx.x;
    if (i < n) out[i] = x[i] / d;
}

hipError_t div_scalar(int64_t n, const double* x, double d, double* out, hipStream_t st) {
    if (n <= 0) return hipSuccess;
    hipLaunchKernelGGL(div_scalar_kernel, dim3((unsigned)cdiv(n, kBlock)), dim3(kBlock), 0, st, n, x, d, out);
    return hipGetLastError();
}

__global__ void div2_scalar_kernel(int64_t n, const double* __restrict__ x, const double* __restrict__ r, double d,
                                   double* __restrict__ out) {
    const int64_t i = (int64_t)blockIdx.x * kBlock + threadIdx.x;
    if (i < n) {
        out[i] = x[i] / d;
        out[n + i] = r[i] / d;
    }
}

hipError_t div2_scalar(int64_t n, const double* x, const double* r, double d, double* out, hipStream_t st) {
    if (n <= 0) return hipSuccess;
    hipLaunchKernelGGL(div2_scalar_kernel, dim3((unsigned)cdiv(n, kBlock)), dim3(kBlock), 0, st, n, x, r, d, out);
    return hipGetLastError();
}

__global__ __launch_bounds__(kBlock) void cg_init_kernel(int K, int64_t M, CgVecs c, double diag, RedOut ro) {
    __shared__ double lds[4];
    double acc[2 * kMaxRhs];
#pragma unroll
    for (int q = 0; q < 2 * kMaxRhs; ++q) acc[q] = 0.0;
    for (int64_t i = (int64_t)blockIdx.x * kBlock + threadIdx.x; i < M; i += (int64_t)gridDim.x * kBlock) {
#pragma unroll
        for (int k = 0; k < kMaxRhs; ++k) {
// ... 17 lines not shown
            }
        }
    }
    block_put_sums<2 * kMaxRhs>(acc, 2 * K, ro, (int64_t)blockIdx.x * 2 * K);
    red_finish(ro, 2 * K, lds);
}

__global__ __launch_bounds__(kBlock) void prelude_cg_init_kernel(int K, int64_t M, Prelude p, CgVecs c, double diag,
                                                                 RedOut ro, CgState start, CgState* dst) {
    __shared__ double lds[4];
    __shared__ double fin[2 * kMaxRhs];
    double eta1 = p.eta1, gam1 = p.gam1, gam2 = p.gam2, gamw = p.gamw, tau = c.tau, cgam2 = c.gam2;
    if (p.dev.scal) {
        const double* q = p.dev.scal;
        eta1 = q[0];
        gam2 = cgam2 = q[1];
        gamw = tau = q[2];
        diag = q[3];
        gam1 = q[4];
    }
    double acc[2 * kMaxRhs];
#pragma unroll
    for (int q = 0; q < 2 * kMaxRhs; ++q) acc[q] = 0.0;
    const int64_t stride = (int64_t)gridDim.x * kBlock;
    for (int64_t i0 = (int64_t)blockIdx.x * kBlock + threadIdx.x; i0 < M; i0 += 2 * stride) {
        const bool two = i0 + stride < M;
        double x1v[2], r1v[2], ayv[2], vo[2][kMaxRhs], a0[2][kMaxRhs], muv[2][kMaxRhs], dd[2][kMaxRhs];
#pragma unroll
        for (int h = 0; h < 2; ++h) {
            const int64_t i = i0 + h * stride;
            if (h == 1 && !two) break;
            x1v[h] = p.x1[i];
            r1v[h] = p.r1[i];
            ayv[h] = p.atxy[i];
#pragma unroll
            for (int k = 0; k < kMaxRhs; ++k) {
                if (k >= K) continue;
                vo[h][k] = c.v[k] == p.v || c.v[k] == p.bern ? 0.0 : c.v[k][i];
                a0[h][k] = c.atx0[k] ? c.atx0[k][i] : 0.0;
                muv[h][k] = c.atx0[k] ? c.mu[k][i] : 0.0;
                dd[h][k] = !c.atx0[k] && c.d[k] ? c.d[k][i] : 0.0;
            }
        }
#pragma unroll
        for (int h = 0; h < 2; ++h) {
            const int64_t i = i0 + h * stride;
            if (h == 1 && !two) break;
            const double r2 = (eta1 * x1v[h] - gam1 * r1v[h]) / gam2;
            p.r2[i] = r2;
            const double vv = gamw * ayv[h] + gam2 * r2;
            p.v[i] = vv;
            const double bn = (double)(2 * bern_bit(p.seed, p.it, p.S + i) - 1) / p.sqrtMt;
            p.bern[i] = bn;
            if (p.bern_next) p.bern_next[i] = (double)(2 * bern_bit(p.seed, p.it + 1, p.S + i) - 1) / p.sqrtMt;
            if (p.zero[0]) p.zero[0][i] = 0.0;
            if (p.zero[1]) p.zero[1][i] = 0.0;
#pragma unroll
            for (int k = 0; k < kMaxRhs; ++k) {
                if (k >= K) continue;
                const double vi = c.v[k] == p.v ? vv : c.v[k] == p.bern ? bn : vo[h][k];
                double r;
                if (c.atx0[k]) {
                    double dv = a0[h][k];
                    dv *= tau;
                    dv += cgam2 * muv[h][k];
                    r = vi - dv;
                } else {
                    r = c.d[k] ? vi - dd[h][k] : vi - 0.0;
                }
                const double z = r / diag;
                c.r[k][i] = r;
                c.z[k][i] = z;
                c.p[k][i] = z;
                acc[2 * k] += r * z;
                acc[2 * k + 1] += vi * vi;
            }
        }
    }
    block_put_sums<2 * kMaxRhs>(acc, 2 * K, ro, (int64_t)blockIdx.x * 2 * K);
    if (red_finish(ro, 2 * K, lds, fin) && dst && threadIdx.x == 0) {
        *dst = start;
        dst->gam2 = cgam2;
        for (int k = 0; k < K; ++k) {
            dst->rz[k] = fin[2 * k];
            dst->vv[k] = fin[2 * k + 1];
        }
    }
}

hipError_t prelude_cg_init(int K, int64_t M, const Prelude& p, const CgVecs& c, double diag, const RedOut& ro,
                           const CgState* start, CgState* dst, hipStream_t st) {
    hipLaunchKernelGGL(prelude_cg_init_kernel, dim3(red_blocks(M)), dim3(kBlock), 0, st, K, M, p, c, diag, ro,
                       start ? *start : CgState{}, start ? dst : nullptr);
    return hipGetLastError();
}

hipError_t cg_init(int K, int64_t M, const CgVecs& c, double diag, const RedOut& ro, hipStream_t st) {
    hipLaunchKernelGGL(cg_init_kernel, dim3(red_blocks(M)), dim3(kBlock), 0, st, K, M, c, diag, ro);
    return hipGetLastError();
}

__global__ void cg_start_kernel(CgState init, CgState* dst) {
    if (threadIdx.x == 0) *dst = init;
}

hipError_t cg_start(const CgState& init, CgState* dst, hipStream_t st) {
    hipLaunchKernelGGL(cg_start_kernel, dim3(1), dim3(64), 0, st, init, dst);
// ... 738 lines not shown
```

vampomi_amd/csrc/pcg.cpp:

```cpp
#include <cstddef>
#include <string>

#include "ctx.h"

template <class T>
static T* field(vk::CgState* cs, size_t off) {
    return reinterpret_cast<T*>(reinterpret_cast<char*>(cs) + off);
}

struct CgOutcome {
    int any = 0;
    bool pre = false;
    int iters[vk::kMaxRhs] = {};
};

static constexpr int kCgPackWord = 2;

static vampomi_status read_packed(vampomi_ctx* c, int step, unsigned long long seq, CgOutcome* o) {
    const int word = kCgPackWord + (step & 1);
    STCHK(wait_flag(c, seq << 32, word));
    STCHK(op_check_err(c));
    const unsigned long long w = __atomic_load_n(c->h_flag + word, __ATOMIC_ACQUIRE);
    if ((w >> 32) != (seq & 0xffffffffULL))
        return fail(VAMPOMI_ERR_STATE, "CG step " + std::to_string(step) + ": decision word holds sequence " +
// ... 222 lines not shown
    unsigned long long token = 0;

    explicit OnePassSolve(const Pcg& s)
        : Pcg(s), hs(a.hs), AR(c->op_nvec), Q(AR + (int64_t)vk::kMaxRhs * c->ld),
          AD(AR + (int64_t)2 * vk::kMaxRhs * c->ld), cu(fill_vecs(s, true)),
          fold(c->use_comm && c->cg_fold && c->opp.T >= 1 && (!head || c->opp_hs.T >= 1)),
          packed(K <= 2 && a.max_iter < vk::kCgPackMaxIter) {
        cu.nA = c->N;
        for (int k = 0; k < K; ++k) {
            cu.Q[k] = Q + (int64_t)k * c->ld;
            cu.AR[k] = head && k == 0 ? hs->abern : AR + (int64_t)k * c->ld;
            cu.AD[k] = AD + (int64_t)k * c->ld;
        }
        if (!c->use_comm) {
            cu.adpart = c->op_part;
            cu.adld = c->ld;
            cu.adslots = c->opp.nslots;
        }
        cu.addiv = c->sqrtN;
    }
    vk::CgState* state(int i) const { return c->cgs + i; }
    vk::OpArgs op_args() const {
        vk::OpArgs o{};
        o.beta = beta();
        o.diag = diag;
        o.tau = a.tau;
        o.gam2 = a.gam2;
        return o;
    }
    void op_system(vk::OpArgs& o, int k) const {
        o.ar.p[k] = cu.AR[k];
        o.qo.p[k] = cu.Q[k];
        o.p.p[k] = sys[k]->p;
        o.z.p[k] = sys[k]->z;
        o.d.p[k] = sys[k]->d;
        o.sraw.p[k] = rec ? sys[k]->S : nullptr;
    }

    vampomi_status first_products() {
        Product pr[vk::kMaxRhs];
        int n = 0;
        bool given = false;
        for (int k = 0; k < K; ++k) {
            if (a.ar0 && a.ar0[k]) {
                given = true;
                STCHK(copy_nvec(c, AR + (int64_t)k * c->ld, a.ar0[k]));
            } else {
                pr[n++] = {sys[k]->r, AR + (int64_t)k * c->ld};
            }
        }
        if (a.extra_x) pr[n++] = {a.extra_x, a.ex_out};
        if (xnext()) pr[n++] = {xnext(), hs->axnext};
        return ax_products(c, n, pr, given ? a.nscratch : AR);
    }

    vampomi_status compose_step() {
        vk::PreCompose pc{};
        pc.T1 = hs->T1;
        pc.U1 = hs->U1;
        pc.ab = cu.AR[0];
        pc.p = sys[0]->p;
        pc.d = sys[0]->d;
        pc.S = rec ? sys[0]->S : nullptr;
        pc.AD = const_cast<double*>(cu.AD[0]);
        pc.diag = diag;
        pc.tau = a.tau;
        pc.gam2 = a.gam2;
        HIPCHK(vk::pre_compose(c->M, c->N, pc, red(SL_DP, gate()), c->st));
        vk::CgVecs cp = cu;
        cp.adpart = nullptr;
        cp.addiv = 0.0;
        vk::CgDecide dc{};
        dc.on = 1;
        dc.it = -2;
        dc.mask = 1;
        HIPCHK(vk::cg_update(1, c->M, cp, diag, c->cgs, c->scal + SL_DP, nullptr, 0, red(SL_CG, gate()), dc,
                             c->st));
        hs->pre_used = true;
        return VAMPOMI_OK;
    }

    vampomi_status head_step() {
        vk::OpArgs o = op_args();
        op_system(o, 0);
        o.fuse = pre2 ? 1 : 0;
        const double* xn = xnext();
        const double* px[vk::kOpPlain] = {sys[1]->r, a.extra_x, xn ? xn : a.extra_x};
        double* out[vk::kOpPlain] = {cu.AR[1], a.ex_out, xn ? hs->axnext : a.nscratch};
        STCHK(op_dev_plain(c, o, px, out, gate()));
        vk::CgVecs ch = cu;
        if (!c->use_comm) ch.adslots = (int)c->opp_hs.nslots;
        else ch.addiv = 0.0;
        const double* dp = c->use_comm ? AD + (int64_t)(1 + vk::kOpPlain) * c->ld : c->scal + SL_DP;
        vk::CgDecide dc{};
        dc.on = !c->use_comm;
        dc.it = -1;
        dc.mask = 1;
        HIPCHK(vk::cg_update(1, c->M, ch, diag, c->cgs, dp, nullptr, pre2 ? 1 : 0, red(SL_CG, gate()), dc,
                             c->st));
        if (c->use_comm) {
            STCHK(allreduce_dev(c, c->scal + SL_CG, 3));
            if (fold) {
                pend.on = 1;
                pend.it = -1;
                pend.mask = 1;
            } else {
                HIPCHK(vk::cg_decide(c->cgs, c->scal + SL_CG, -1, nullptr, nullptr, 0, c->st, 1));
            }
        }
        hs->used = true;
        return VAMPOMI_OK;
    }

    vampomi_status enqueue(int i, unsigned long long* seq) {
        const int fuse = i > 0 ? (1 << K) - 1 : head ? 1 : 0;
        vk::OpArgs o = op_args();
        for (int k = 0; k < K; ++k) op_system(o, k);
        if (offer) {
            o.alt.cs = c->cgs;
            o.alt.done = hs->pre_done;
            o.alt.token = token;
            o.alt.ar = hs->axnext;
            o.alt.p = hs->xnext;
            o.alt.d = hs->T1;
        }
        o.fuse = fuse;
        const int* g = gate();
        vk::CgState* cs = c->cgs;
        if (fold) {
            o.beta = nullptr;
            if (pend.on) {
                o.fold = pend;
                o.fold.src = state(cur);
                o.fold.dst = state(cur ^ 1);
                o.fold.red = c->scal + SL_CG;
                cur ^= 1;
                pend.on = 0;
            }
            cs = state(cur);
            g = field<int>(cs, offsetof(vk::CgState, any));
            if (!o.fold.on) o.beta = field<double>(cs, offsetof(vk::CgState, beta));
        }
        STCHK(op_dev(c, K, o, g, c->use_comm, false));
        const double* dp = c->use_comm ? AD + (int64_t)K * c->ld : c->scal + SL_DP;
        *seq = ++c->sync_seq;
        unsigned long long* flag = packed ? c->d_flag + kCgPackWord + (i & 1) : c->d_flag;
        vk::CgMirror* mirror = packed ? nullptr : c->d_cgm;
        vk::CgDecide dc{};
        if (!c->use_comm) {
            dc.on = 1;
            dc.it = i;
            dc.mirror = mirror;
            dc.flag = flag;
            dc.seq = *seq;
            dc.pack = packed ? 1 : 0;
        }
        HIPCHK(vk::cg_update(K, c->M, cu, diag, cs, dp, nullptr, fuse, red(SL_CG, g), dc, c->st));
        if (c->use_comm) {
            STCHK(allreduce_dev(c, c->scal + SL_CG, (size_t)(3 * K)));
            if (fold) {
                pend.on = 1;
                pend.it = i;
                pend.mask = 0xf;
                pend.pack = packed ? 1 : 0;
                pend.mirror = mirror;
                pend.flag = flag;
                pend.seq = *seq;
            } else {
                HIPCHK(vk::cg_decide(c->cgs, c->scal + SL_CG, i, mirror, flag, *seq, c->st, 0xf, packed ? 1 : 0));
            }
        }
        return VAMPOMI_OK;
    }

    vampomi_status settle() {
        if (!pend.on) return VAMPOMI_OK;
        HIPCHK(vk::cg_decide(state(cur), c->scal + SL_CG, pend.it, pend.mirror, pend.flag, pend.seq, c->st, pend.mask,
                             pend.pack));
        pend.on = 0;
        return VAMPOMI_OK;
    }

    vampomi_status finish(const CgOutcome& last) {
        STCHK(op_check_err(c));
        store_iters(*this, last);
        if (offer) hs->pre_made = last.pre;
        return VAMPOMI_OK;
    }

    vampomi_status run() {
        if (!head) STCHK(first_products());
        if (pre2) STCHK(compose_step());
        if (head) STCHK(head_step());
        offer = pre_ok && packed && hs->pre_offer && hs->xnext && hs->axnext && !fold;
        if (offer) {
            token = ++c->pre_seq;
            cu.pre_u1 = hs->U1;
            cu.pre_done = hs->pre_done;
            cu.pre_token = token;
        }
        CgOutcome last;
        STCHK(cg_loop(c, a.max_iter, packed, *this, &last));
        return finish(last);
    }
};

struct TwoPassSolve : Pcg {
    vk::CgVecs cu;
    double* dd[vk::kMaxRhs];
    double* ss[vk::kMaxRhs];
    const bool split_dp;

    explicit TwoPassSolve(const Pcg& s)
        : Pcg(s), cu(fill_vecs(s, true)), split_dp(c->use_comm && K < vk::kMaxRhs && !c->dp_separate) {
        for (int k = 0; k < K; ++k) {
            dd[k] = sys[k]->d;
            ss[k] = sys[k]->S;
            cu.AS[k] = a.nscratch + (int64_t)k * c->ld;
            if (sys[k]->AW) cu.nA = c->N;
        }
    }

    vampomi_status enqueue(int i, unsigned long long* seq) {
        const bool fuse = i > 0;
        vk::AxFuse fu{};
        fu.gate = gate();
        if (fuse) {
            for (int k = 0; k < K; ++k) fu.z.p[k] = cu.z[k];
            fu.beta = beta();
        }
        const double* px[vk::kMaxRhs];
        for (int k = 0; k < K; ++k) px[k] = cu.p[k];
        const bool ex = i == 0 && a.extra_x;
        if (ex) px[K] = a.extra_x;
        const int KA = ex ? K + 1 : K;
        const double* pp_dev = nullptr;
        vk::DotArgs tail{};
        if (split_dp) {
            tail.nt = K;
            for (int k = 0; k < K; ++k)
                tail.t[k] = fuse ? vk::DotTerm{cu.p[k], cu.p[k], vk::SQPUPD, cu.z[k], beta() + k}
                                 : vk::DotTerm{cu.p[k], cu.p[k], vk::DOT};
            pp_dev = a.nscratch + (int64_t)KA * c->ld;
        }
        STCHK(ax_dev(c, KA, px, a.nscratch, &fu, split_dp ? &tail : nullptr));
        if (ex) STCHK(copy_nvec(c, a.ex_out, a.nscratch + (int64_t)K * c->ld));
        if (split_dp) {
// ... 51 lines not shown
```

vampomi_amd/csrc/run.h:

```cpp
#pragma once
#include <string>
#include <vector>

#include "ctx.h"
#include "writer.h"

struct Mixture {
    int L = 0;
    double probs[VAMPOMI_MAX_L] = {};
    double vars[VAMPOMI_MAX_L] = {};
};

inline double smax(double a, double b) { return (a < b) ? b : a; }
inline double smin(double a, double b) { return (b < a) ? b : a; }

struct VampRun {
    vampomi_params prm{};
    vampomi_result* res = nullptr;
    bool probit = false;
    bool write = false;
    bool fuse = true;
    bool recur = false;
    bool arec = false;
    bool onepass = false;
    int z1n_slot = 2;
    int bern_it = 0;
    int abern_it = 0;
    int em_head = 0, z_head = 0;
    double zh_bsum = 0, zh_cnt[4] = {}, zh_xc[3] = {};
    int hs_it = 0;
    std::string out_dir, out_name, p_params, p_metrics, p_prior;
    int it = 0;
    bool stopped = false;
    bool io_err = false;
    std::string io_msg;
    IterWriter* writer = nullptr;
    Mixture mix, mix_next;
    bool have_next = false;
    double gam1 = 0, gam2 = 0, gamw = 0;
    double alpha1 = 0, alpha2 = 0, eta1 = 0, eta2 = 0, alpha1_next = 0;
    double metrics[12] = {}, params[8] = {};
    double e1m[3] = {}, e1n[2] = {}, e1s[3] = {}, e2m[3] = {}, e2n[2] = {}, e2s[3] = {};
    double tn = 0, tc = 0, nm[2] = {}, sum_d = 0, a2 = 0;
    double *r1 = nullptr, *x1 = nullptr, *x1p = nullptr, *x1n = nullptr, *x1d = nullptr, *r2 = nullptr;
    double *x2 = nullptr, *bern = nullptr, *invQ = nullptr, *v = nullptr, *atxy = nullptr, *ts = nullptr;
    double *tmpM = nullptr, *atx0 = nullptr;
    double* cgw[10] = {};
    double *z1buf = nullptr, *nb3 = nullptr , *nsc = nullptr;
    double* ax2 = nullptr;
    double* abern = nullptr;
    double* bern_next = nullptr;
    double* pre_t1 = nullptr;
    double* pre_u1 = nullptr;
    int pre_it = 0;
    double* mixw = nullptr;
    double* mixh = nullptr;
    double* mixh_dev = nullptr;
    bool mix_pending = false;
    Mixture mix_expect;
    int pre_ahead = 0;
    bool pre_ahead_on = true;
    const double* z1 = nullptr;
    int64_t passes_ref = 0;
    double tau1 = 0, tau2 = 0, beta1 = 0, beta2 = 0;
    double* p1 = nullptr;
    double* p2 = nullptr;
    double* z1h = nullptr;
    double* x1s = nullptr;
    double* x1sn = nullptr;
    double* x2s = nullptr;
    double* prior_row = nullptr;
    double ph_solve_s = 0, ph_step_s = 0;

    ~VampRun();
};

struct EmParams {
    int EM_max_iter;
    double EM_err_thr;
    int learn_vars;
    double merge_vars_thr;
    int verbosity;
};
EmParams em_params(const VampRun& R);
vampomi_status update_prior(vampomi_ctx* c, const EmParams& P, Mixture& m, double gam1, const double* r1);
vampomi_status update_prior(vampomi_ctx* c, const VampRun& R, Mixture& m, double gam1, const double* r1);
struct EmState {
    int emit = 0;
    double lambda = 0;
    double omegas[VAMPOMI_MAX_L] = {};
    double sums[2 * VAMPOMI_MAX_L] = {};
};
struct R1From {
    const double* x2;
    const double* r2;
    double eta2, gam2, gam1;
    const double* dsc = nullptr;
};
vampomi_status em_begin(vampomi_ctx* c, const EmParams& P, const Mixture& m, double gam1, const double* r1,
                        DotBatch& b, EmState& s, const R1From* r1from = nullptr, const vk::EmUpd* upd = nullptr);
vampomi_status em_queue(vampomi_ctx* c, const Mixture& m, double gam1, const double* r1, DotBatch& b, EmState& s,
                        const R1From* r1from = nullptr, const vk::EmUpd* upd = nullptr);
vampomi_status em_finish(vampomi_ctx* c, const EmParams& P, Mixture& m, double gam1, const double* r1, EmState& s);
vampomi_status denoise_into(vampomi_ctx* c, const Mixture& m, double gam1, const double* r1, double* x1,
                            const double* x1_prev, bool damp, double rho, double* x1d, DotBatch& b, double* sum_out,
                            const double* mixw = nullptr, const double* gam1dev = nullptr,
                            const vk::PreOut* po = nullptr);
vampomi_status upload_or_zero(vampomi_ctx* c, double* dst, const double* host, int64_t n);
vampomi_status write_bins(vampomi_ctx* c, VampRun& R);
void write_row(VampRun& R, const std::string& path, int it, const double* vals, int n);
vampomi_status agree_io(vampomi_ctx* c, VampRun& R, bool wait_all = false);
vampomi_status end_iteration_io(vampomi_ctx* c, VampRun& R);
vampomi_status probit_begin(vampomi_ctx* c, VampRun& R);
// ... 2 lines not shown
```

vampomi_amd/csrc/vamp.cpp:

```cpp
#include <algorithm>
#include <chrono>
#include <cmath>
#include <cstdio>
#include <cstring>

#include "ctx.h"
#include "hostio.h"
#include "run.h"

VampRun::~VampRun() {
    if (writer) writer->drain(nullptr);
    for (double** p : {&r1, &x1, &x1p, &x1n, &x1d, &r2, &x2, &bern, &invQ, &v, &atxy, &ts, &tmpM, &atx0, &z1buf,
                       &nb3, &nsc, &ax2, &p1, &p2, &z1h, &x1s, &x1sn, &x2s, &abern, &bern_next, &pre_t1, &pre_u1})
        dev_free(*p);
    for (auto& p : cgw) dev_free(p);
    dev_free(mixw);
    if (mixh) (void)hipHostFree(mixh);
}

vampomi_ctx::vampomi_ctx() = default;

vampomi_ctx::~vampomi_ctx() {
    run.reset();
    writer.reset();
// ... 131 lines not shown
                       double* s3, std::vector<DotBatch::Group>& gm, std::vector<DotBatch::Group>& gn) {
    gm.push_back({{T(xhat, R.ts), T(xhat, xhat), T(R.ts, R.ts)}, true, m3});
    gn.push_back({{T(c->y, Axest, vk::DIFF2), T(c->y, c->y)}, false, n2});
    gn.push_back({{T(Axest, c->y), T(Axest, Axest), T(c->y, c->y)}, true, s3});
}

static vampomi_status err_queue(vampomi_ctx* c, VampRun& R, const double* xhat, const double* Axest, DotBatch& b,
                                double* m3, double* n2, double* s3, std::vector<DotBatch::Group> gm = {},
                                std::vector<DotBatch::Group> gn = {}) {
    err_groups(c, R, xhat, Axest, m3, n2, s3, gm, gn);
    STCHK(b.add_many(c->M, gm));
    return b.add_many(c->N, gn);
}

static void err_finish(VampRun& R, const double* m3, const double* n2, const double* s3, int ind) {
    const double corr = m3[0] / std::sqrt(m3[1] * m3[2]);
    const double l2_pred_err = std::sqrt(n2[0] / n2[1]);
    const double R2 = 1 - l2_pred_err * l2_pred_err;
    const double corr_y = s3[0] / std::sqrt(s3[1] * s3[2]);
    const double corr_y_2 = corr_y * corr_y;
    if (ind == 1) {
        R.metrics[1] = corr;
        R.metrics[0] = R2;
        R.metrics[4] = corr_y_2;
    } else {
        R.metrics[3] = corr;
        R.metrics[2] = R2;
        R.metrics[5] = corr_y_2;
    }
}

vampomi_status upload_or_zero(vampomi_ctx* c, double* dst, const double* host, int64_t n) {
    if (n <= 0) return VAMPOMI_OK;
    if (host)
        HIPCHK(hipMemcpyAsync(dst, host, (size_t)n * 8, hipMemcpyHostToDevice, c->st));
    else
        HIPCHK(hipMemsetAsync(dst, 0, (size_t)n * 8, c->st));
    return VAMPOMI_OK;
}

static bool keeps_hist(const VampRun& R) { return R.res && (R.res->x1_hist || R.res->r1_hist); }
vampomi_status ensure_writer(vampomi_ctx* c, VampRun& R);

static vampomi_status vamp_alloc(vampomi_ctx* c, VampRun& R) {
    const size_t M = (size_t)std::max<int64_t>(c->M, 1), ld = (size_t)c->ld;
    for (double** p : {&R.r1, &R.x1, &R.x1p, &R.x1n, &R.x1d, &R.r2, &R.x2, &R.bern, &R.invQ, &R.v, &R.atxy, &R.ts,
                       &R.tmpM, &R.atx0, &R.bern_next})
        STCHK(dev_alloc(p, M));
    for (auto& p : R.cgw) STCHK(dev_alloc(&p, M));
    STCHK(dev_alloc(&R.z1buf, ld));
    STCHK(dev_alloc(&R.nb3, vk::kMaxRhs * ld));
    STCHK(dev_alloc(&R.nsc, vk::kMaxRhs * ld));
    STCHK(dev_alloc(&R.ax2, ld));
    STCHK(dev_alloc(&R.abern, 2 * ld));
    STCHK(dev_alloc(&R.pre_t1, M));
    STCHK(dev_alloc(&R.pre_u1, ld + 2));
    HIPCHK(hipMemsetAsync(R.pre_t1, 0, M * 8, c->st));
    HIPCHK(hipMemsetAsync(R.pre_u1, 0, (ld + 2) * 8, c->st));
    STCHK(dev_alloc(&R.mixw, vk::kMixWords));
    HIPCHK(hipHostMalloc((void**)&R.mixh, (vk::kMixWords + 4) * sizeof(double),
                         hipHostMallocMapped | hipHostMallocCoherent));
    {
        const char* e = std::getenv("VAMPOMI_PRE_AHEAD");
        R.pre_ahead_on = !e || std::atoi(e) != 0;
    }
    HIPCHK(hipHostGetDevicePointer((void**)&R.mixh_dev, R.mixh, 0));
    HIPCHK(hipMemsetAsync(R.ax2, 0, ld * 8, c->st));
    HIPCHK(hipMemsetAsync(R.abern, 0, 2 * ld * 8, c->st));
    HIPCHK(hipMemsetAsync(R.z1buf, 0, ld * 8, c->st));
    HIPCHK(hipMemsetAsync(R.nb3, 0, vk::kMaxRhs * ld * 8, c->st));
    HIPCHK(hipMemsetAsync(R.nsc, 0, vk::kMaxRhs * ld * 8, c->st));
    return VAMPOMI_OK;
}

extern "C" vampomi_status vampomi_vamp_begin(vampomi_ctx* c, const vampomi_params* p, vampomi_result* r) {
    CollScope cs_(c);
    if (!c || !p) return fail(VAMPOMI_ERR_ARG, "null argument");
    if (!c->have_X || !c->have_y) return fail(VAMPOMI_ERR_STATE, "load methylation data and phenotype first");
    const bool probit = p->model && std::strcmp(p->model, "bin_class") == 0;
    if (p->model && !probit && std::strcmp(p->model, "linear") != 0)
        return fail(VAMPOMI_ERR_MODEL, std::string("Invalid model specification! ('") + p->model + "')");
    if (p->L < 1 || p->L > VAMPOMI_MAX_L) return fail(VAMPOMI_ERR_ARG, "number of mixture components out of range");
    HIPCHK(hipSetDevice(c->device));
    STCHK(op_agree(c));
    c->run.reset(new VampRun());
    c->pre_made_n = c->pre_used_n = 0;
    VampRun& R = *c->run;
    R.prm = *p;
    R.res = r;
    R.probit = probit;
    R.fuse = p->batch_rhs != 0;
    R.recur = p->batch_rhs >= 2;
    R.arec = p->batch_rhs >= 3;
    R.onepass = p->batch_rhs >= 4;
    R.out_dir = p->out_dir ? p->out_dir : "";
    R.out_name = p->out_name ? p->out_name : "";
    R.write = !R.out_dir.empty();
    R.mix.L = p->L;
    for (int j = 0; j < p->L; ++j) {
        R.mix.probs[j] = p->probs[j];
        R.mix.vars[j] = p->vars[j] * (double)c->N;
    }
    R.gam1 = p->gam1;
    R.gamw = 1.0 / (1.0 - p->h2);
    R.gam2 = 0;
    STCHK(vamp_alloc(c, R));
    if (R.write || keeps_hist(R)) STCHK(ensure_writer(c, R));
    STCHK(upload_or_zero(c, R.ts, p->true_signal, c->M));
    std::vector<double> h((size_t)std::max<int64_t>(c->M, 1), 0.0);
    for (int64_t i = 0; i < c->M; ++i) h[i] = (p->x1hat_init ? p->x1hat_init[i] : 0.0) / std::sqrt((double)c->N);
    STCHK(upload_or_zero(c, R.x1, h.data(), c->M));
    STCHK(upload_or_zero(c, R.r1, h.data(), c->M));
    STCHK(upload_or_zero(c, R.x2, nullptr, c->M));
    if (R.probit) {
        if (r) {
            r->iterations_run = 0;
            r->a_passes_ref = 0;
            r->a_passes_exec = 0;
        }
        STCHK(probit_begin(c, R));
        STCHK(sync_stream(c, c->st));
// ... 99 lines not shown
    if (R.writer && R.writer->failed(&msg)) return fail(VAMPOMI_ERR_HIP, msg);
    return VAMPOMI_OK;
}

static vampomi_status check_device_mix(VampRun& R) {
    if (!R.mix_pending) return VAMPOMI_OK;
    R.mix_pending = false;
    const Mixture& m = R.mix_expect;
    bool same = (double)m.L == R.mixh[0];
    for (int j = 0; same && j < m.L; ++j)
        same = std::memcmp(&m.probs[j], &R.mixh[1 + j], 8) == 0 &&
               std::memcmp(&m.vars[j], &R.mixh[1 + vk::kMaxL + j], 8) == 0;
    if (!same) return fail(VAMPOMI_ERR_STATE, "vamp: the device's EM update differs from the host's");
    return VAMPOMI_OK;
}

struct LmmseSetup {
    CgSystem sx{}, so{};
    bool rec = false, arec = false, hs_av = false, pre_in_cg = false;
    HeadStart hs;
    vk::Prelude pr{};
};

static vampomi_status lmmse_setup(vampomi_ctx* c, VampRun& R, int it, const double* x1, LmmseSetup& L) {
    const int64_t ld = c->ld;
    CgSystem& sx = L.sx;
    CgSystem& so = L.so;
    sx.v = R.v;
    sx.mu = R.x2;
    sx.mu0_nonzero = it > 1;
    sx.atx0 = (it > 1 && R.have_next) ? R.atx0 : nullptr;
    sx.r = R.cgw[0];
    sx.z = R.cgw[1];
    sx.p = R.cgw[2];
    sx.d = R.cgw[3];
    so.v = R.bern;
    so.mu = R.invQ;
    so.onsager = true;
    so.r = R.cgw[4];
    so.z = R.cgw[5];
    so.p = R.cgw[6];
    so.d = R.cgw[7];
    L.rec = R.recur && R.fuse && (it == 1 || sx.atx0);
    if (L.rec) {
        sx.W = R.atx0;
        sx.S = R.cgw[8];
        so.W = R.tmpM;
        so.S = R.cgw[9];
    }
    L.arec = R.arec && L.rec;
    if (L.arec) sx.AW = R.ax2;
    if (R.fuse && L.arec && R.onepass) STCHK(headstart_available(c, &L.hs_av));
    if (L.hs_av) {
        L.hs.abern = R.hs_it == it ? R.abern + (it & 1) * ld : nullptr;
        if (it < R.prm.max_iter) {
            L.hs.xnext = R.bern_next;
            L.hs.axnext = R.abern + ((it + 1) & 1) * ld;
        }
        if (prestep_on(c)) {
            L.hs.T1 = R.pre_t1;
            L.hs.U1 = R.pre_u1;
            L.hs.pre_done = reinterpret_cast<unsigned long long*>(R.pre_u1 + ld);
            L.hs.pre_have = L.hs.abern && R.pre_it == it;
            L.hs.pre_offer = L.hs.xnext != nullptr;
        }
    }
    vk::Prelude& pr = L.pr;
    pr.eta1 = R.eta1;
    pr.gam1 = R.gam1;
    pr.gam2 = R.gam2;
    pr.gamw = R.gamw;
    pr.x1 = x1;
    pr.r1 = R.r1;
    pr.atxy = R.atxy;
    pr.r2 = R.r2;
    pr.v = R.v;
    pr.seed = R.prm.seed;
    pr.it = it;
    pr.S = c->S;
    pr.sqrtMt = std::sqrt((double)c->Mt);
    pr.bern = R.bern;
    pr.bern_next = L.hs.xnext ? R.bern_next : nullptr;
    pr.zero[0] = R.invQ;
    pr.zero[1] = L.rec ? R.tmpM : nullptr;
    L.pre_in_cg = R.fuse && (L.hs_av || L.arec);
    return VAMPOMI_OK;
}

static vampomi_status check_device_values(vampomi_ctx* c, VampRun& R, int it) {
    STCHK(check_device_mix(R));
    if (R.pre_ahead != it) return VAMPOMI_OK;
    R.pre_ahead = 0;
    const double diag = R.gamw * (double)(c->N - 1) / (double)c->N + R.gam2;
    const double want[4] = {R.eta1, R.gam2, R.gamw, diag};
    if (std::memcmp(want, R.mixh + vk::kMixWords, sizeof want) != 0)
        return fail(VAMPOMI_ERR_STATE, "vamp: the prelude queued ahead formed other scalars than the host");
    return VAMPOMI_OK;
}

extern "C" vampomi_status vampomi_vamp_step(vampomi_ctx* c, int* stopped) {
    CollScope cs_(c);
    if (!c || !c->run) return fail(VAMPOMI_ERR_STATE, "vampomi_vamp_begin not called");
    VampRun& R = *c->run;
    if (R.stopped || R.it >= R.prm.max_iter) {
        R.stopped = true;
        if (stopped) *stopped = 1;
        return VAMPOMI_OK;
    }
    HIPCHK(hipSetDevice(c->device));
    const auto t_step = std::chrono::steady_clock::now();
    if (R.probit) {
        STCHK(probit_step(c, R));
        R.ph_step_s = std::chrono::duration<double>(std::chrono::steady_clock::now() - t_step).count();
        if (c->timing) resolve_timing(c);
        if (stopped) *stopped = R.stopped ? 1 : 0;
        return VAMPOMI_OK;
    }
    const int64_t M = c->M, N = c->N, Mt = c->Mt, ld = c->ld;
    const int it = ++R.it;
    vampomi_result* res = R.res;

    if (!R.have_next) {
        if (it > R.prm.learn_prior_delay) STCHK(update_prior(c, R, R.mix, R.gam1, R.r1));
        std::swap(R.x1, R.x1p);
        DotBatch b(c);
        STCHK(denoise_into(c, R.mix, R.gam1, R.r1, R.x1, R.x1p, it > 1, R.prm.rho, R.x1d, b, &R.sum_d));
        STCHK(b.flush());
        R.alpha1 = R.sum_d / (double)Mt;
        if (!R.arec) {
            const double* xs[1] = {R.x1};
            STCHK(ax_dev(c, 1, xs, R.z1buf));
        }
        R.z1 = R.z1buf;
    } else {
        double* old = R.x1p;
        R.x1p = R.x1;
        R.x1 = R.x1n;
        R.x1n = old;
        R.mix = R.mix_next;
        R.alpha1 = R.alpha1_next;
        R.z1 = R.arec ? R.z1buf : R.nb3 + R.z1n_slot * ld;
    }
    R.passes_ref += 1;
    if (res && res->L_hist) res->L_hist[it - 1] = R.mix.L;
    R.eta1 = R.gam1 / R.alpha1;
    STCHK(write_bins(c, R));
    R.gam2 = smin(smax(R.eta1 - R.gam1, 1e-11), 1e11);
    DotBatch e1(c);
    if (!R.arec) STCHK(err_queue(c, R, R.x1, R.z1, e1, R.e1m, R.e1n, R.e1s));
    R.params[0] = R.alpha1;
    R.params[1] = R.gam1;

    R.passes_ref += 1;
    LmmseSetup L;
    STCHK(lmmse_setup(c, R, it, R.x1, L));
    CgSystem& sx = L.sx;
    CgSystem& so = L.so;
    const bool rec = L.rec, arec = L.arec, hs_av = L.hs_av;
    HeadStart& hs = L.hs;
    vk::Prelude& pr = L.pr;
    if (it == 1) {
        HIPCHK(hipMemsetAsync(R.x2, 0, (size_t)std::max<int64_t>(M, 1) * 8, c->st));
        if (rec) HIPCHK(hipMemsetAsync(R.atx0, 0, (size_t)std::max<int64_t>(M, 1) * 8, c->st));
        if (arec) HIPCHK(hipMemsetAsync(R.ax2, 0, (size_t)ld * 8, c->st));
    }
    const PreMode pm = R.pre_ahead == it ? PreMode::queued : PreMode::normal;
    if (pm == PreMode::queued && !(L.pre_in_cg && R.fuse && hs_av))
        return fail(VAMPOMI_ERR_STATE, "vamp: the start queued ahead does not match this iteration's schedule");
    if (!L.pre_in_cg) HIPCHK(vk::prelude(M, pr, c->st));
    const auto t_solve = std::chrono::steady_clock::now();
    PcgArgs pargs;
    pargs.tau = R.gamw;
    pargs.gam2 = R.gam2;
    pargs.max_iter = R.prm.CG_max_iter;
    pargs.tol = R.prm.CG_err_tol;
    pargs.nscratch = R.nsc;
    pargs.ref_passes = &R.passes_ref;
    if (R.fuse && hs_av) {
        pargs.extra_x = R.x1;
        pargs.ex_out = R.z1buf;
        pargs.onepass = true;
        pargs.hs = &hs;
        pargs.pre = &pr;
        pargs.pm = pm;
        STCHK(pcg_run(c, {&so, &sx}, pargs));
        R.hs_it = hs.xnext ? it + 1 : 0;
        R.pre_it = hs.pre_made ? it + 1 : 0;
        c->pre_made_n += hs.pre_made ? 1 : 0;
        c->pre_used_n += hs.pre_used ? 1 : 0;
    } else if (R.fuse) {
        if (arec) {
            pargs.extra_x = R.x1;
            pargs.ex_out = R.z1buf;
            pargs.pre = &pr;
        } else {
            pargs.init = &e1;
        }
        pargs.onepass = R.onepass;
        STCHK(pcg_run(c, {&sx, &so}, pargs));
        R.hs_it = R.pre_it = 0;
    } else {
        R.pre_it = 0;
        PcgArgs first = pargs;
        first.init = &e1;
        STCHK(pcg_run(c, {&sx}, first));
        STCHK(pcg_run(c, {&so}, pargs));
    }
    R.ph_solve_s = std::chrono::duration<double>(std::chrono::steady_clock::now() - t_solve).count();
    STCHK(check_device_values(c, R, it));
    if (res && res->cg_iters) res->cg_iters[it - 1] = sx.iters;
    if (res && res->ons_iters) res->ons_iters[it - 1] = so.iters;
    const bool next = R.fuse && it < R.prm.max_iter;
    const bool em_next = next && it + 1 > R.prm.learn_prior_delay;
    const bool r1_in_em = next && arec && em_next && R.prm.EM_max_iter >= 1;
    const bool chain = r1_in_em && (!c->use_comm || c->mr_tail);
    const bool mr = chain && c->use_comm;
    const DotBatch::Group ga2{{T(R.bern, R.invQ)}, true, &R.a2};
    const double gam1_prev = R.gam1;
    auto host_gam1 = [&] {
        R.alpha2 = R.gam2 * R.a2;
        err_finish(R, R.e1m, R.e1n, R.e1s, 1);
        R.eta2 = R.gam2 / R.alpha2;
        R.gam1 = smin(smax(R.eta2 - R.gam2, 1e-11), 1e11);
        R.gam1 = R.prm.rho * R.gam1 + (1 - R.prm.rho) * gam1_prev;
    };
    DotBatch fin(c);
    double* dsc = c->scal + SL_CHAIN;
    const DotBatch::Group gtc{{T(R.bern, R.tmpM)}, true, &R.tc};
    const DotBatch::Group gtn{{T(R.ax2, c->y, vk::DIFF2)}, false, &R.tn};
    const DotBatch::Group gnm{{T(R.x1p, R.x1, vk::DIFF2), T(R.x1p, R.x1p)}, true, R.nm};
    if (chain) {
        std::vector<DotBatch::Group> gm{ga2}, gn;
        err_groups(c, R, R.x1, R.z1, R.e1m, R.e1n, R.e1s, gm, gn);
        gm.push_back(gtc);
        gm.push_back(gnm);
        gn.push_back(gtn);
        err_groups(c, R, R.x2, R.ax2, R.e2m, R.e2n, R.e2s, gm, gn);
        vk::G1Chain g1;
        g1.gam2 = R.gam2;
        g1.rho = R.prm.rho;
        g1.gam1_prev = gam1_prev;
        g1.out = dsc;
        if (!mr) {
            STCHK(fin.add_pair(M, gm, &g1, &R.a2, {{&R.tc, dsc + 9}}, N, gn, {{&R.tn, dsc + 8}}));
        } else {
            STCHK(fin.add_pair(M, gm, nullptr, nullptr, {}, N, gn, {}));
            STCHK(fin.reduce_now());
            vk::TailPost t;
            t.mode = 0;
            t.src = fin.dev_slot(&R.a2);
            t.g1 = g1;
            t.cp_src[0] = fin.dev_slot(&R.tc);
            t.cp_dst[0] = dsc + 9;
// ... 76 lines not shown

    const double* ax2 = R.nb3;
    bool shared = false;
    if (arec) {
        ax2 = R.ax2;
        R.passes_ref += 3;
        shared = true;
    } else if (rec) {
        const double* xs[2] = {R.x2, R.x1n};
        STCHK(ax_dev(c, next ? 2 : 1, xs, R.nb3));
        R.z1n_slot = 1;
        R.passes_ref += 2;
        STCHK(fin.add({T(R.nb3, c->y, vk::DIFF2)}, N, false, &R.tn));
        R.passes_ref += 1;
        STCHK(fin.add({T(R.bern, R.tmpM)}, M, true, &R.tc));
    } else {
        const double* xs[3] = {R.x2, R.invQ, R.x1n};
        STCHK(ax_dev(c, next ? 3 : 2, xs, R.nb3));
        R.z1n_slot = 2;
        R.passes_ref += 2;
        STCHK(fin.add({T(R.nb3, c->y, vk::DIFF2)}, N, false, &R.tn));
        const double* u[2] = {R.nb3 + ld, R.nb3};
        double* o[2] = {R.tmpM, R.atx0};
        STCHK(atx_dev(c, next ? 2 : 1, u, o, 0, 0.0, 0.0, nullptr));
        R.passes_ref += 1;
        STCHK(fin.add({T(R.bern, R.tmpM)}, M, true, &R.tc));
    }
    if (shared && !chain)
        STCHK(err_queue(c, R, R.x2, ax2, fin, R.e2m, R.e2n, R.e2s, {gtc, gnm}, {gtn}));
    else if (!shared)
        STCHK(err_queue(c, R, R.x2, ax2, fin, R.e2m, R.e2n, R.e2s));
    R.passes_ref += 1;
    if (next && arec && em_next && !devem) {
        STCHK(fin.flush());
        if (chain) host_gam1();
        STCHK(em_finish(c, em_params(R), R.mix_next, R.gam1, R.r1, em));
    }
    if (next && arec && !devem)
        STCHK(denoise_into(c, R.mix_next, R.gam1, R.r1, R.x1n, R.x1, true, R.prm.rho, R.x1d, fin, &R.sum_d));
    if (!shared) STCHK(fin.add_many(M, {gnm}));
    if (ahead) {
        PcgArgs pargs;
        pargs.max_iter = R.prm.CG_max_iter;
        pargs.tol = R.prm.CG_err_tol;
        pargs.nscratch = R.nsc;
        pargs.extra_x = R.x1n;
        pargs.ex_out = R.z1buf;
        pargs.onepass = true;
        pargs.hs = &A.hs;
        pargs.pre = &A.pr;
        pargs.pm = PreMode::ahead;
        STCHK(pcg_run(c, {&A.so, &A.sx}, pargs));
        R.pre_ahead = it + 1;
    }
    STCHK(fin.flush());
    if (devem) {
        host_gam1();
        STCHK(em_finish(c, em_params(R), R.mix_next, R.gam1, R.r1, em));
        R.mix_expect = R.mix_next;
        R.mix_pending = true;
    }
    const double trace_corr = R.tc * (double)Mt;
    if (R.prm.verbosity >= 1 && c->rank == 0)
        std::printf("l2_norm2(temp) / N = %g\ntrace_correction / N = %g\n", R.tn / (double)N, trace_corr / (double)N);
    R.gamw = (double)N / (R.tn + trace_corr);
    err_finish(R, R.e2m, R.e2n, R.e2s, 2);
    R.params[2] = R.alpha2;
    R.params[3] = R.gam2;
    R.params[4] = R.gamw;
    if (res && res->params) std::memcpy(res->params + (int64_t)(it - 1) * 5, R.params, 5 * sizeof(double));
    if (res && res->metrics) std::memcpy(res->metrics + (int64_t)(it - 1) * 6, R.metrics, 6 * sizeof(double));
    if (R.write && c->rank == 0) {
        write_row(R, R.p_params, it, R.params, 5);
        write_row(R, R.p_metrics, it, R.metrics, 6);
    }
    if (R.prm.verbosity >= 1 && c->rank == 0)
        std::printf("it %d: alpha1 %.6g gam1 %.6g alpha2 %.6g gam2 %.6g gamw %.6g L %d cg %d/%d\n", it, R.alpha1,
                    R.gam1, R.alpha2, R.gam2, R.gamw, R.mix.L, sx.iters, so.iters);

    const double NMSE = std::sqrt(R.nm[0] / R.nm[1]);
    if ((it > 1 && NMSE < R.prm.stop_criteria_thr) || it >= R.prm.max_iter) R.stopped = true;
    STCHK(end_iteration_io(c, R));
    R.have_next = next && !R.stopped;
    if (R.have_next) R.alpha1_next = R.sum_d / (double)Mt;
    if (res) {
        res->iterations_run = it;
        res->a_passes_ref = R.passes_ref;
        res->a_passes_exec = c->stats.a_passes_exec;
    }
    if (c->timing) resolve_timing(c);
    if (stopped) *stopped = R.stopped ? 1 : 0;
    R.ph_step_s = std::chrono::duration<double>(std::chrono::steady_clock::now() - t_step).count();
    return VAMPOMI_OK;
}

extern "C" vampomi_status vampomi_step_phases(vampomi_ctx* c, double* solve_s, double* step_s) {
    if (!c || !c->run) return fail(VAMPOMI_ERR_STATE, "vampomi_vamp_begin not called");
    if (solve_s) *solve_s = c->run->ph_solve_s;
    if (step_s) *step_s = c->run->ph_step_s;
    return VAMPOMI_OK;
}

extern "C" vampomi_status vampomi_vamp_end(vampomi_ctx* c) {
    if (!c || !c->run) return fail(VAMPOMI_ERR_STATE, "vampomi_vamp_begin not called");
    VampRun& R = *c->run;
    vampomi_result* res = R.res;
// ... 104 lines not shown
```

Measured before the change: 183.7.

## Fold the CG pre-step into a widened two-system head-start operator kernel

Adds a K=2 form of the plain head-start team kernel. During the head-start pass it also computes the first product of the next iteration's Bernoulli probe system and writes that extra partial into an enlarged part buffer, which the reduce kernel then sums into U1. The Bernoulli/abern buffers become a three-deep ring so the probe for the iteration after next can be computed a step early. The aim is to drop a separate pre-step A pass by sharing the matrix read. In exchange there is more register pressure, smaller S limits, extra buffer memory, and a one-time bootstrap A·x when the ring is not yet primed.

```diff
diff --git a/include/vampomi.h b/include/vampomi.h
--- a/include/vampomi.h
+++ b/include/vampomi.h
@@ -171,6 +171,8 @@
                                    int* grid, int* nslots, char* name, int cap);
 vampomi_status vampomi_dev_op_plan(int64_t N, int64_t M, int cus, int variant, int K, int* T, int* S, int* TR,
                                    int* grid, int64_t* nslots, char* name, int cap);
+vampomi_status vampomi_dev_op_head_plan(int64_t N, int64_t M, int cus, int variant, int* T, int* S, int* TR,
+                                        int* wide, int64_t* lds, char* name, int cap);
 vampomi_status vampomi_dev_op_lds(int64_t N, int64_t M, int cus, int variant, int K, int64_t* out);
 vampomi_status vampomi_dev_op_timestamps(vampomi_ctx* ctx, unsigned long long* out, int cap, int* n);
 vampomi_status vampomi_dev_mem_plan(int64_t N, int64_t Mt, int nranks, int rank, int cus, int probit, int writer,
diff --git a/vampomi_amd/_lib.py b/vampomi_amd/_lib.py
--- a/vampomi_amd/_lib.py
+++ b/vampomi_amd/_lib.py
@@ -136,6 +136,8 @@
     "vampomi_dev_op_plan": (C.c_int, [C.c_int64, C.c_int64, C.c_int, C.c_int, C.c_int, _P, _P, _P, _P, _P, C.c_char_p,
                                       C.c_int]),
     "vampomi_dev_op_lds": (C.c_int, [C.c_int64, C.c_int64, C.c_int, C.c_int, C.c_int, _P]),
+    "vampomi_dev_op_head_plan": (C.c_int, [C.c_int64, C.c_int64, C.c_int, C.c_int, _P, _P, _P, _P, _P, C.c_char_p,
+                                           C.c_int]),
     "vampomi_dev_op_apply": (C.c_int, [_P, C.c_int, _P, _P, _P, _P, _P, C.c_double, C.c_double, C.c_double, _P, _P,
                                        _P]),
     "vampomi_dev_op_timestamps": (C.c_int, [_P, _P, C.c_int, C.POINTER(C.c_int)]),
diff --git a/vampomi_amd/csrc/atax_team.hip b/vampomi_amd/csrc/atax_team.hip
--- a/vampomi_amd/csrc/atax_team.hip
+++ b/vampomi_amd/csrc/atax_team.hip
@@ -221,11 +221,15 @@
         return;
     }
     const double* beta = a.fold.on ? s_beta : a.beta;
-    static_assert(K + KP <= kMaxRhs, "partial slots per team");
+    constexpr bool WIDE = K + KP > kMaxRhs;
+    static_assert(!WIDE || (K == 2 && K + KP == kMaxRhs + 1), "partial slots per team");
     int fuse = a.fuse, alt = -1;
     if constexpr (KP == 0) {
         if (a.alt.cs && !a.fold.on) alt = cg_pre_slot(a.alt.cs->active, K, *a.alt.done == a.alt.token);
         if (alt >= 0) fuse &= ~(1 << alt);
+    } else if constexpr (K == 2) {
+        alt = 1;
+        fuse &= ~2;
     }
 #if TM_TS
     const unsigned long long ts0 = __builtin_amdgcn_s_memrealtime();
@@ -633,6 +637,7 @@
         }
     }
     double* dst = a.part + (int64_t)team * kMaxRhs * ld + r0;
+    constexpr int KP0 = WIDE ? 1 : K;
 #pragma unroll
     for (int s = 0; s < S; ++s) {
         const int jl = RS * s + jb;
@@ -641,13 +646,20 @@
         for (int k = 0; k < K; ++k)
 #pragma unroll
             for (int e = 0; e < E; ++e)
-                if (jl + e < nrows) dst[(int64_t)k * ld + jl + e] = acc[k][s][e];
+                if (jl + e < nrows) {
+                    if constexpr (WIDE) {
+                        double* xdst = a.part + ((int64_t)nteams * kMaxRhs + team) * ld + r0;
+                        (k == 1 ? xdst : dst)[jl + e] = acc[k][s][e];
+                    } else {
+                        dst[(int64_t)k * ld + jl + e] = acc[k][s][e];
+                    }
+                }
         if constexpr (KP > 0) {
 #pragma unroll
             for (int k = 0; k < KP; ++k)
 #pragma unroll
                 for (int e = 0; e < E; ++e)
-                    if (jl + e < nrows) dst[(int64_t)(K + k) * ld + jl + e] = accp[k][s][e];
+                    if (jl + e < nrows) dst[(int64_t)(KP0 + k) * ld + jl + e] = accp[k][s][e];
         }
     }
     if constexpr (COMM) {
@@ -687,6 +699,14 @@
                                                                      const double* __restrict__ msig, OpArgs a, int T,
                                                                      int TR, int ilv, const int* __restrict__ gate) {
     atax_team_body<1, S, F, L, P, COMM, E, FMA, kTmPlain>(X, ld, N, M, mave, msig, a, T, TR, ilv, gate);
+}
+template <int S, int F, int L, int P, bool COMM, int E, bool FMA>
+__global__ __launch_bounds__(kTmThreads) void atax_team_plain2_kernel(const double* __restrict__ X, int64_t ld,
+                                                                      int64_t N, int64_t M,
+                                                                      const double* __restrict__ mave,
+                                                                      const double* __restrict__ msig, OpArgs a, int T,
+                                                                      int TR, int ilv, const int* __restrict__ gate) {
+    atax_team_body<2, S, F, L, P, COMM, E, FMA, kTmPlain>(X, ld, N, M, mave, msig, a, T, TR, ilv, gate);
 }
 
 #ifndef AX_TEAM_SYNC
@@ -845,10 +865,12 @@
 static hipError_t launch_tm(const Shard& s, const OpPlan& pl, const OpArgs& a, hipStream_t st, const Timing& tm,
                             const int* gate, int* occ) {
     constexpr TmCfg c = kTmCfg[C];
-    static_assert(!PL || K == 1, "the head-start kernel has one operator system");
+    static_assert(!PL || K <= 2, "the head-start kernel has one operator system, its widened form two");
     void (*kern)(const double*, int64_t, int64_t, int64_t, const double*, const double*, OpArgs, int, int, int,
                  const int*);
-    if constexpr (PL)
+    if constexpr (PL && K == 2)
+        kern = atax_team_plain2_kernel<S, c.F, c.L, c.P, c.comm, c.E, (bool)TM_FMA>;
+    else if constexpr (PL)
         kern = atax_team_plain_kernel<S, c.F, c.L, c.P, c.comm, c.E, (bool)TM_FMA>;
     else
         kern = atax_team_kernel<K, S, c.F, c.L, c.P, c.comm, c.E, (bool)TM_FMA>;
@@ -869,11 +891,14 @@
 static constexpr int tm_plain_maxS(int cfg) {
     return cfg == 0 ? 8 : cfg == 2 ? 3 : cfg == 3 ? 4 : cfg == 4 ? 5 : 0;
 }
+static constexpr int tm_plain2_maxS(int cfg) {
+    return cfg == 0 ? 6 : cfg == 2 ? 3 : cfg == 3 ? 4 : cfg == 4 ? 4 : 0;
+}
 
 template <int K, int C, int S, bool PL>
 static hipError_t launch_tm_if(const Shard& s, const OpPlan& pl, const OpArgs& a, hipStream_t st, const Timing& tm,
                                const int* gate, int* occ) {
-    if constexpr (S <= (PL ? tm_plain_maxS(C) : kTmCfg[C].maxS))
+    if constexpr (S <= (PL ? (K == 2 ? tm_plain2_maxS(C) : tm_plain_maxS(C)) : kTmCfg[C].maxS))
         return launch_tm<K, S, C, PL>(s, pl, a, st, tm, gate, occ);
     return hipErrorInvalidValue;
 }
@@ -910,10 +935,10 @@
     const OpArgs a = tm_with_slots(a0, K);
     if constexpr (PL) {
         switch (pl.cfg) {
-            case 0: return launch_tm_s<1, 0, true>(pl.S, s, pl, a, st, tm, gate, occ);
-            case 2: return launch_tm_s<1, 2, true>(pl.S, s, pl, a, st, tm, gate, occ);
-            case 3: return launch_tm_s<1, 3, true>(pl.S, s, pl, a, st, tm, gate, occ);
-            case 4: return launch_tm_s<1, 4, true>(pl.S, s, pl, a, st, tm, gate, occ);
+            case 0: return launch_tm_s<K, 0, true>(pl.S, s, pl, a, st, tm, gate, occ);
+            case 2: return launch_tm_s<K, 2, true>(pl.S, s, pl, a, st, tm, gate, occ);
+            case 3: return launch_tm_s<K, 3, true>(pl.S, s, pl, a, st, tm, gate, occ);
+            case 4: return launch_tm_s<K, 4, true>(pl.S, s, pl, a, st, tm, gate, occ);
             default: return hipErrorInvalidValue;
         }
     }
@@ -945,14 +970,21 @@
 }
 
 hipError_t atax_team_plain(const Shard& s, const OpPlan& pl, const OpArgs& a, hipStream_t st, const Timing& tm,
-                           const int* gate) {
+                           const int* gate, bool wide) {
     if (pl.T < 1 || pl.grid < pl.T || pl.grid % pl.T) return hipErrorInvalidValue;
     if (pl.T > 1 && (!a.xg || !a.err || a.tag == 0)) return hipErrorInvalidValue;
     for (int k = 0; k < kTmPlain; ++k)
         if (!a.px.p[k]) return hipErrorInvalidValue;
+    if (wide && (!team_plain_wide(pl) || !a.alt.ar || !a.alt.p || !a.alt.d || a.fold.on)) return hipErrorInvalidValue;
     if (s.M <= 0) return hipSuccess;
-    if (const hipError_t e = launch_tm_c<1, true>(s, pl, a, st, tm, gate)) return e;
+    const hipError_t e =
+        wide ? launch_tm_c<2, true>(s, pl, a, st, tm, gate) : launch_tm_c<1, true>(s, pl, a, st, tm, gate);
+    if (e != hipSuccess) return e;
     return hipGetLastError();
+}
+
+bool team_plain_wide(const OpPlan& pl) {
+    return pl.T >= 1 && pl.cfg >= 0 && pl.cfg < kTmNCfg && pl.S >= 1 && pl.S <= tm_plain2_maxS(pl.cfg);
 }
 
 bool ax_team_plan(int64_t N, int64_t M, int cus, AxPlan* out) {
@@ -1059,6 +1091,7 @@
         case 1: e = launch_tm_c<1>(s, pl, a, nullptr, Timing{}, nullptr, &occ); break;
         case 2: e = launch_tm_c<2>(s, pl, a, nullptr, Timing{}, nullptr, &occ); break;
         case 1 + kTmPlain: e = launch_tm_c<1, true>(s, pl, a, nullptr, Timing{}, nullptr, &occ); break;
+        case 2 + kTmPlain: e = launch_tm_c<2, true>(s, pl, a, nullptr, Timing{}, nullptr, &occ); break;
         default: break;
     }
     return e == hipSuccess ? occ : 0;
@@ -1067,9 +1100,9 @@
 std::string team_kernel_name(int K, const OpPlan& pl) {
     const TmCfg& c = kTmCfg[pl.cfg];
     char b[128];
-    if (K == 1 + kTmPlain)
-        std::snprintf(b, sizeof b, "atax_team_plain_kernel<%d, %d, %d, %d, %s, %d>", pl.S, c.F, c.L, c.P,
-                      c.comm ? "true" : "false", c.E);
+    if (K == 1 + kTmPlain || K == 2 + kTmPlain)
+        std::snprintf(b, sizeof b, "atax_team_plain%s_kernel<%d, %d, %d, %d, %s, %d>", K == 2 + kTmPlain ? "2" : "",
+                      pl.S, c.F, c.L, c.P, c.comm ? "true" : "false", c.E);
     else
         std::snprintf(b, sizeof b, "atax_team_kernel<%d, %d, %d, %d, %d, %s, %d>", K, pl.S, c.F, c.L, c.P,
                       c.comm ? "true" : "false", c.E);
diff --git a/vampomi_amd/csrc/ctx.h b/vampomi_amd/csrc/ctx.h
--- a/vampomi_amd/csrc/ctx.h
+++ b/vampomi_amd/csrc/ctx.h
@@ -120,6 +120,7 @@
     bool hs_ok = false;
     bool hs_on = true;
     bool hs_on_req = true;
+    bool hs_wide_ok = false;
     int pre_mode = 2;
     unsigned long long pre_seq = 0;
     int64_t pre_made_n = 0, pre_used_n = 0;
@@ -231,6 +232,8 @@
     bool pre_offer = false;
     bool pre_made = false;
     bool pre_used = false;
+    bool pre_head = false;
+    const double* abnext = nullptr;
 };
 enum class PreMode { normal, ahead, queued };
 struct PcgArgs {
@@ -254,9 +257,10 @@
 vampomi_status headstart_available(vampomi_ctx* c, bool* yes);
 constexpr int64_t kPreMinBytes = (int64_t)256 << 20;
 bool prestep_on(const vampomi_ctx* c);
+vampomi_status prestep_head(const vampomi_ctx* c, bool* yes);
 unsigned* op_err_dev(vampomi_ctx* c);
 vampomi_status op_check_err(vampomi_ctx* c);
 vampomi_status op_dev(vampomi_ctx* c, int K, const vk::OpArgs& a, const int* gate, bool reduce = true,
                       bool divide = true);
 vampomi_status op_dev_plain(vampomi_ctx* c, const vk::OpArgs& a, const double* const* px, double* const* out,
-                            const int* gate);
+                            const int* gate, double* u1 = nullptr);
diff --git a/vampomi_amd/csrc/engine.cpp b/vampomi_amd/csrc/engine.cpp
--- a/vampomi_amd/csrc/engine.cpp
+++ b/vampomi_amd/csrc/engine.cpp
@@ -681,6 +681,12 @@
     return (size_t)(Mx + p.grid) * vk::kOpMaxK * (size_t)p.T * 2 + (size_t)p.grid * (2 * vk::kOpMaxK + 1);
 }
 
+static int64_t op_part_rows(const vk::OpPlan& op, const vk::OpPlan* hs) {
+    int64_t rows = op.nslots * vk::kMaxRhs;
+    if (hs) rows = std::max<int64_t>(rows, hs->nslots * (vk::kMaxRhs + (vk::team_plain_wide(*hs) ? 1 : 0)));
+    return rows;
+}
+
 static vampomi_status op_plan_local(vampomi_ctx* c) {
     if (c->cus <= 0) HIPCHK(hipDeviceGetAttribute(&c->cus, hipDeviceAttributeMultiprocessorCount, c->device));
     const int64_t M = std::max<int64_t>(c->M, 1);
@@ -698,6 +704,8 @@
     }
     bool hs_ok = op_ok && vk::team_plain_plan(c->N, M, c->cus, c->opp, &c->opp_hs);
     if (hs_ok && (int64_t)vk::team_occupancy(c->opp_hs, 1 + vk::kOpPlain) * c->cus < c->opp_hs.grid) hs_ok = false;
+    c->hs_wide_ok = hs_ok && vk::team_plain_wide(c->opp_hs) &&
+                    (int64_t)vk::team_occupancy(c->opp_hs, 2 + vk::kOpPlain) * c->cus >= c->opp_hs.grid;
     c->op_ok_mine = op_ok;
     c->hs_ok_mine = hs_ok;
     if (!c->op_ts && std::getenv("VAMPOMI_OP_TS") && std::atoi(std::getenv("VAMPOMI_OP_TS"))) {
@@ -709,10 +717,10 @@
         HIPCHK(hipMemsetAsync(c->op_nvec, 0, ((size_t)3 * vk::kMaxRhs * c->ld + 16) * 8, c->st));
     }
     if (op_ok) {
-        const int64_t slots = std::max<int64_t>(c->opp.nslots, hs_ok ? c->opp_hs.nslots : 0);
+        const int64_t slots = op_part_rows(c->opp, hs_ok ? &c->opp_hs : nullptr);
         if (slots > c->op_part_slots) {
             dev_free(c->op_part);
-            STCHK(dev_alloc(&c->op_part, (size_t)slots * vk::kMaxRhs * c->ld));
+            STCHK(dev_alloc(&c->op_part, (size_t)slots * c->ld));
             c->op_part_slots = slots;
         }
         if (c->opp.T > 1 || (hs_ok && c->opp_hs.T > 1)) {
@@ -882,10 +890,13 @@
 }
 
 vampomi_status op_dev_plain(vampomi_ctx* c, const vk::OpArgs& a, const double* const* px, double* const* out,
-                            const int* gate) {
+                            const int* gate, double* u1) {
     if (!c->have_X) return fail(VAMPOMI_ERR_STATE, "A before the methylation data was loaded");
     STCHK(op_prepare(c));
     if (!c->hs_ok) return fail(VAMPOMI_ERR_ARG, "head-start launch: no plan for N = " + std::to_string(c->N));
+    if (u1 && (c->use_comm || !c->hs_wide_ok))
+        return fail(VAMPOMI_ERR_ARG, "head-start launch: no widened form of " +
+                                         vk::team_kernel_name(1 + vk::kOpPlain, c->opp_hs) + " on this context");
     constexpr int KT = 1 + vk::kOpPlain;
     double* ad = c->op_nvec + (int64_t)2 * vk::kMaxRhs * c->ld;
     vk::OpArgs x = a;
@@ -901,15 +912,18 @@
     x.dbg = 0;
     x.ro = vk::RedOut{c->red_part, c->use_comm ? ad + (int64_t)KT * c->ld : c->scal + SL_DP, c->ticket, nullptr, 0,
                       gate};
-    TimedLaunch t = launch_stat(c, 3, KT, pass_bytes(c, KT), pass_flops(c, 1) + pass_flops(c, KT));
+    TimedLaunch t = launch_stat(c, 3, KT, pass_bytes(c, KT + (u1 ? 1 : 0)),
+                                pass_flops(c, 1) + pass_flops(c, KT) + (u1 ? 2.0 * pass_flops(c, 1) : 0.0));
     STCHK(team_launch(c, c->opp_hs.T, [&] {
-        return vk::atax_team_plain(c->shard(), c->opp_hs, x, c->st, vk::Timing{t.a, t.b}, gate);
+        return vk::atax_team_plain(c->shard(), c->opp_hs, x, c->st, vk::Timing{t.a, t.b}, gate, u1 != nullptr);
     }));
     c->stats.a_passes_exec++;
     if (!c->use_comm) {
         vk::Ptrs os{};
         for (int k = 0; k < vk::kOpPlain; ++k) os.p[k] = out[k];
-        HIPCHK(vk::op_reduce(c->opp_hs, vk::kOpPlain, c->N, c->ld, c->op_part, os, c->sqrtN, c->st, gate, 1));
+        const double* xpart = u1 ? c->op_part + c->opp_hs.nslots * vk::kMaxRhs * c->ld : nullptr;
+        HIPCHK(vk::op_reduce(c->opp_hs, vk::kOpPlain, c->N, c->ld, c->op_part, os, c->sqrtN, c->st, gate, 1, xpart,
+                             u1));
     } else {
         vk::Ptrs os{};
         for (int k = 0; k < KT; ++k) os.p[k] = ad + (int64_t)k * c->ld;
@@ -1057,7 +1071,7 @@
     if (const char* hv = std::getenv("VAMPOMI_HEADSTART")) c->hs_on = c->hs_on_req = std::atoi(hv) != 0;
     if (const char* pv = std::getenv("VAMPOMI_PRESTEP")) {
         const int v = std::atoi(pv);
-        if (v >= 0 && v <= 2) c->pre_mode = v;
+        if (v >= 0 && v <= 3) c->pre_mode = v;
     }
     const char* mode = std::getenv("VAMPOMI_COMM");
     if (c->use_comm && mode && std::strcmp(mode, "loopback") == 0) {
@@ -1624,7 +1638,7 @@
         c->hs_on_req = variant == 1;
         if (!c->use_comm) c->hs_on = c->hs_on_req;
     } else if (which == 7) {
-        if (variant < 0 || variant > 2) return fail(VAMPOMI_ERR_ARG, "pre-step: 0, 1 or 2");
+        if (variant < 0 || variant > 3) return fail(VAMPOMI_ERR_ARG, "pre-step: 0, 1, 2 or 3");
         c->pre_mode = variant;
     } else if (which == 6) {
         if (variant != 0 && variant != 1) return fail(VAMPOMI_ERR_ARG, "multi-rank tail: 0 or 1");
@@ -1639,7 +1653,16 @@
 
 bool prestep_on(const vampomi_ctx* c) {
     if (c->use_comm || c->nranks != 1 || !c->hs_ok || c->pre_mode == 0) return false;
-    return c->pre_mode == 1 || std::max<int64_t>(c->M, 1) * c->ld * 8 >= kPreMinBytes;
+    return c->pre_mode != 2 || std::max<int64_t>(c->M, 1) * c->ld * 8 >= kPreMinBytes;
+}
+
+vampomi_status prestep_head(const vampomi_ctx* c, bool* yes) {
+    *yes = prestep_on(c) && c->pre_mode >= 2 && c->hs_wide_ok;
+    if (prestep_on(c) && c->pre_mode == 3 && !c->hs_wide_ok)
+        return fail(VAMPOMI_ERR_ARG, "pre-step in the head-start launch (VAMPOMI_PRESTEP=3): the head-start plan " +
+                                         vk::team_kernel_name(1 + vk::kOpPlain, c->opp_hs) + " (T = " +
+                                         std::to_string(c->opp_hs.T) + ") has no widened form");
+    return VAMPOMI_OK;
 }
 
 extern "C" vampomi_status vampomi_dev_prestep_counts(const vampomi_ctx* c, int64_t* made, int64_t* used) {
@@ -1800,6 +1823,23 @@
     return VAMPOMI_OK;
 }
 
+extern "C" vampomi_status vampomi_dev_op_head_plan(int64_t N, int64_t M, int cus, int variant, int* T, int* S,
+                                                   int* TR, int* wide, int64_t* lds, char* name, int cap) {
+    vk::OpPlan p{}, h{};
+    const int64_t Mx = std::max<int64_t>(M, 1);
+    if (!vk::op_plan(N, Mx, cus, variant, &p) || !vk::team_plain_plan(N, Mx, cus, p, &h))
+        return fail(VAMPOMI_ERR_ARG, "no head-start plan");
+    const bool w = vk::team_plain_wide(h);
+    if (T) *T = h.T;
+    if (S) *S = h.S;
+    if (TR) *TR = h.TR;
+    if (wide) *wide = w ? 1 : 0;
+    if (lds && !vk::team_lds_layout(h, N, w ? 2 : 1, lds)) return fail(VAMPOMI_ERR_ARG, "no LDS layout");
+    if (name && cap > 0)
+        std::snprintf(name, (size_t)cap, "%s", vk::team_kernel_name((w ? 2 : 1) + vk::kOpPlain, h).c_str());
+    return VAMPOMI_OK;
+}
+
 extern "C" vampomi_status vampomi_dev_op_lds(int64_t N, int64_t M, int cus, int variant, int K, int64_t* out) {
     vk::OpPlan p{};
     if (!out || !vk::op_plan(N, std::max<int64_t>(M, 1), cus, variant, &p) || !vk::team_lds_layout(p, N, K, out))
@@ -1832,14 +1872,14 @@
     if (vk::op_plan(N, Mx, cus, vk::kOpDefault, &op)) {
         const bool h = vk::team_plain_plan(N, Mx, cus, op, &hs);
         add((int64_t)3 * vk::kMaxRhs * ld + 16, 8);
-        add(std::max<int64_t>(op.nslots, h ? hs.nslots : 0) * vk::kMaxRhs * ld, 8);
+        add(op_part_rows(op, h ? &hs : nullptr) * ld, 8);
         size_t w = op.T > 1 ? op_xg_words_for(Mx, op) : 0;
         if (h && hs.T > 1) w = std::max(w, op_xg_words_for(Mx, hs));
         if (w) add((int64_t)w, 8);
     }
     for (int q = 0; q < 25; ++q) add(Mx, 8);
     add(ld, 8), add((int64_t)vk::kMaxRhs * ld, 8), add((int64_t)vk::kMaxRhs * ld, 8), add(ld, 8);
-    add(2 * ld, 8);
+    add(3 * ld, 8);
     add(Mx, 8), add(ld + 2, 8);
     if (probit) {
         for (int q = 0; q < 3; ++q) add(ld, 8);
@@ -1858,7 +1898,8 @@
     if (K == 1 + vk::kOpPlain) {
         vk::OpPlan h{};
         if (!vk::team_plain_plan(c->N, std::max<int64_t>(c->M, 1), cus, p, &h)) return "(no head-start plan)";
-        return vk::team_kernel_name(K, h);
+        const bool wide = prestep_on(c) && c->pre_mode >= 2 && c->hs_wide_ok && vk::team_plain_wide(h);
+        return vk::team_kernel_name(wide ? K + 1 : K, h);
     }
     return vk::op_kernel_name(K, p);
 }
diff --git a/vampomi_amd/csrc/kernels.h b/vampomi_amd/csrc/kernels.h
--- a/vampomi_amd/csrc/kernels.h
+++ b/vampomi_amd/csrc/kernels.h
@@ -146,10 +146,12 @@
 hipError_t atax_team(const Shard& s, const OpPlan& pl, int K, const OpArgs& a, hipStream_t st, const Timing& tm,
                      const int* gate);
 hipError_t atax_team_plain(const Shard& s, const OpPlan& pl, const OpArgs& a, hipStream_t st, const Timing& tm,
-                           const int* gate);
+                           const int* gate, bool wide = false);
+bool team_plain_wide(const OpPlan& pl);
 bool team_plain_plan(int64_t N, int64_t M, int cus, const OpPlan& main, OpPlan* out);
 hipError_t op_reduce(const OpPlan& pl, int K, int64_t N, int64_t ld, const double* part, Ptrs out, double div,
-                     hipStream_t st, const int* gate = nullptr, int k0 = 0);
+                     hipStream_t st, const int* gate = nullptr, int k0 = 0, const double* xpart = nullptr,
+                     double* xout = nullptr);
 
 hipError_t marker_stats(const double* X, int64_t ld, int64_t N, int64_t M, double nonas,
                         double alpha_scale, double* mave, double* msig, hipStream_t st);
@@ -265,6 +267,7 @@
     double sqrtMt;
     double* bern;
     double* bern_next;
+    int ahead;
     double* zero[2];
 };
 hipError_t prelude(int64_t M, const Prelude& p, hipStream_t st);
diff --git a/vampomi_amd/csrc/kernels.hip b/vampomi_amd/csrc/kernels.hip
--- a/vampomi_amd/csrc/kernels.hip
+++ b/vampomi_amd/csrc/kernels.hip
@@ -1034,7 +1034,9 @@
 
 __global__ __launch_bounds__(256) void op_reduce_kernel(int64_t N, int64_t ld, int nslots,
                                                         const double* __restrict__ part, Ptrs out, double div,
-                                                        const int* __restrict__ gate) {
+                                                        const int* __restrict__ gate, int K,
+                                                        const double* __restrict__ xpart,
+                                                        double* __restrict__ xout) {
     if (gate && !*gate) return;
     __shared__ v2d wsum[4][64];
     const int lane = threadIdx.x & 63, w = threadIdx.x >> 6;
@@ -1042,24 +1044,26 @@
     const int k = (int)(blockIdx.x / tpk);
     const int64_t i = (blockIdx.x - k * tpk) * 128 + 2 * lane;
     const bool ok = i < N;
-    wsum[w][lane] = ok ? slot_sum(part + (int64_t)k * ld + i, (int64_t)kMaxRhs * ld, w * nslots / 4,
-                                  (w + 1) * nslots / 4)
+    const bool ext = k >= K;
+    const double* src = ext ? xpart + i : part + (int64_t)k * ld + i;
+    wsum[w][lane] = ok ? slot_sum(src, ext ? ld : (int64_t)kMaxRhs * ld, w * nslots / 4, (w + 1) * nslots / 4)
                        : v2d{0.0, 0.0};
     __syncthreads();
     if (w != 0 || !ok) return;
     v2d r = ((wsum[0][lane] + wsum[1][lane]) + wsum[2][lane]) + wsum[3][lane];
     if (div > 0) r /= div;
-    out.p[k][i] = r.x;
-    if (i + 1 < N) out.p[k][i + 1] = r.y;
+    double* o = ext ? xout : out.p[k];
+    o[i] = r.x;
+    if (i + 1 < N) o[i + 1] = r.y;
 }
 
 hipError_t op_reduce(const OpPlan& pl, int K, int64_t N, int64_t ld, const double* part, Ptrs out, double div,
-                     hipStream_t st, const int* gate, int k0) {
+                     hipStream_t st, const int* gate, int k0, const double* xpart, double* xout) {
     const int64_t n = (int64_t)K * N;
     if (n <= 0) return hipSuccess;
-    if (k0 < 0 || k0 + K > kMaxRhs) return hipErrorInvalidValue;
-    hipLaunchKernelGGL(op_reduce_kernel, dim3((unsigned)(K * cdiv(N, 128))), dim3(256), 0, st, N, ld, (int)pl.nslots,
-                       part + (int64_t)k0 * ld, out, div, gate);
+    if (k0 < 0 || k0 + K > kMaxRhs || (xout && !xpart)) return hipErrorInvalidValue;
+    hipLaunchKernelGGL(op_reduce_kernel, dim3((unsigned)((K + (xout ? 1 : 0)) * cdiv(N, 128))), dim3(256), 0, st, N, ld,
+                       (int)pl.nslots, part + (int64_t)k0 * ld, out, div, gate, K, xpart, xout);
     return hipGetLastError();
 }
 
@@ -1591,7 +1595,7 @@
     p.r2[i] = r2;
     p.v[i] = p.gamw * p.atxy[i] + p.gam2 * r2;
     p.bern[i] = (double)(2 * bern_bit(p.seed, p.it, p.S + i) - 1) / p.sqrtMt;
-    if (p.bern_next) p.bern_next[i] = (double)(2 * bern_bit(p.seed, p.it + 1, p.S + i) - 1) / p.sqrtMt;
+    if (p.bern_next) p.bern_next[i] = (double)(2 * bern_bit(p.seed, p.it + 1 + p.ahead, p.S + i) - 1) / p.sqrtMt;
     if (p.zero[0]) p.zero[0][i] = 0.0;
     if (p.zero[1]) p.zero[1][i] = 0.0;
 }
@@ -1715,7 +1719,8 @@
             p.v[i] = vv;
             const double bn = (double)(2 * bern_bit(p.seed, p.it, p.S + i) - 1) / p.sqrtMt;
             p.bern[i] = bn;
-            if (p.bern_next) p.bern_next[i] = (double)(2 * bern_bit(p.seed, p.it + 1, p.S + i) - 1) / p.sqrtMt;
+            if (p.bern_next)
+                p.bern_next[i] = (double)(2 * bern_bit(p.seed, p.it + 1 + p.ahead, p.S + i) - 1) / p.sqrtMt;
             if (p.zero[0]) p.zero[0][i] = 0.0;
             if (p.zero[1]) p.zero[1][i] = 0.0;
 #pragma unroll
diff --git a/vampomi_amd/csrc/pcg.cpp b/vampomi_amd/csrc/pcg.cpp
--- a/vampomi_amd/csrc/pcg.cpp
+++ b/vampomi_amd/csrc/pcg.cpp
@@ -298,6 +298,12 @@
         if (a.extra_x) pr[n++] = {a.extra_x, a.ex_out};
         if (xnext()) pr[n++] = {xnext(), hs->axnext};
         return ax_products(c, n, pr, given ? a.nscratch : AR);
+    }
+
+    void alt_system(vk::OpArgs& o) const {
+        o.alt.ar = hs->abnext ? hs->abnext : hs->axnext;
+        o.alt.p = hs->xnext;
+        o.alt.d = hs->T1;
     }
 
     vampomi_status compose_step() {
@@ -333,7 +339,10 @@
         const double* xn = xnext();
         const double* px[vk::kOpPlain] = {sys[1]->r, a.extra_x, xn ? xn : a.extra_x};
         double* out[vk::kOpPlain] = {cu.AR[1], a.ex_out, xn ? hs->axnext : a.nscratch};
-        STCHK(op_dev_plain(c, o, px, out, gate()));
+        const bool wide = pre_ok && packed && !fold && hs->pre_head && hs->pre_offer && hs->abnext && xn;
+        if (wide) alt_system(o);
+        STCHK(op_dev_plain(c, o, px, out, gate(), wide ? hs->U1 : nullptr));
+        hs->pre_made = wide;
         vk::CgVecs ch = cu;
         if (!c->use_comm) ch.adslots = (int)c->opp_hs.nslots;
         else ch.addiv = 0.0;
@@ -366,9 +375,7 @@
             o.alt.cs = c->cgs;
             o.alt.done = hs->pre_done;
             o.alt.token = token;
-            o.alt.ar = hs->axnext;
-            o.alt.p = hs->xnext;
-            o.alt.d = hs->T1;
+            alt_system(o);
         }
         o.fuse = fuse;
         const int* g = gate();
@@ -438,7 +445,7 @@
         if (!head) STCHK(first_products());
         if (pre2) STCHK(compose_step());
         if (head) STCHK(head_step());
-        offer = pre_ok && packed && hs->pre_offer && hs->xnext && hs->axnext && !fold;
+        offer = pre_ok && packed && hs->pre_offer && hs->xnext && hs->axnext && !fold && !hs->pre_made;
         if (offer) {
             token = ++c->pre_seq;
             cu.pre_u1 = hs->U1;
diff --git a/vampomi_amd/csrc/run.h b/vampomi_amd/csrc/run.h
--- a/vampomi_amd/csrc/run.h
+++ b/vampomi_amd/csrc/run.h
@@ -29,6 +29,7 @@
     int em_head = 0, z_head = 0;
     double zh_bsum = 0, zh_cnt[4] = {}, zh_xc[3] = {};
     int hs_it = 0;
+    int hs2_it = 0;
     std::string out_dir, out_name, p_params, p_metrics, p_prior;
     int it = 0;
     bool stopped = false;
@@ -59,6 +60,7 @@
     bool mix_pending = false;
     Mixture mix_expect;
     int pre_ahead = 0;
+    int pre_ahead_look = 0;
     bool pre_ahead_on = true;
     const double* z1 = nullptr;
     int64_t passes_ref = 0;
diff --git a/vampomi_amd/csrc/vamp.cpp b/vampomi_amd/csrc/vamp.cpp
--- a/vampomi_amd/csrc/vamp.cpp
+++ b/vampomi_amd/csrc/vamp.cpp
@@ -207,7 +207,7 @@
     STCHK(dev_alloc(&R.nb3, vk::kMaxRhs * ld));
     STCHK(dev_alloc(&R.nsc, vk::kMaxRhs * ld));
     STCHK(dev_alloc(&R.ax2, ld));
-    STCHK(dev_alloc(&R.abern, 2 * ld));
+    STCHK(dev_alloc(&R.abern, 3 * ld));
     STCHK(dev_alloc(&R.pre_t1, M));
     STCHK(dev_alloc(&R.pre_u1, ld + 2));
     HIPCHK(hipMemsetAsync(R.pre_t1, 0, M * 8, c->st));
@@ -221,7 +221,7 @@
     }
     HIPCHK(hipHostGetDevicePointer((void**)&R.mixh_dev, R.mixh, 0));
     HIPCHK(hipMemsetAsync(R.ax2, 0, ld * 8, c->st));
-    HIPCHK(hipMemsetAsync(R.abern, 0, 2 * ld * 8, c->st));
+    HIPCHK(hipMemsetAsync(R.abern, 0, 3 * ld * 8, c->st));
     HIPCHK(hipMemsetAsync(R.z1buf, 0, ld * 8, c->st));
     HIPCHK(hipMemsetAsync(R.nb3, 0, vk::kMaxRhs * ld * 8, c->st));
     HIPCHK(hipMemsetAsync(R.nsc, 0, vk::kMaxRhs * ld * 8, c->st));
@@ -427,10 +427,13 @@
     if (L.arec) sx.AW = R.ax2;
     if (R.fuse && L.arec && R.onepass) STCHK(headstart_available(c, &L.hs_av));
     if (L.hs_av) {
-        L.hs.abern = R.hs_it == it ? R.abern + (it & 1) * ld : nullptr;
+        bool ph = false;
+        if (prestep_on(c)) STCHK(prestep_head(c, &ph));
+        L.hs.abern = R.hs_it == it ? R.abern + (it % 3) * ld : nullptr;
         if (it < R.prm.max_iter) {
             L.hs.xnext = R.bern_next;
-            L.hs.axnext = R.abern + ((it + 1) & 1) * ld;
+            L.hs.axnext = R.abern + ((it + (ph ? 2 : 1)) % 3) * ld;
+            if (ph) L.hs.abnext = R.abern + ((it + 1) % 3) * ld;
         }
         if (prestep_on(c)) {
             L.hs.T1 = R.pre_t1;
@@ -438,6 +441,7 @@
             L.hs.pre_done = reinterpret_cast<unsigned long long*>(R.pre_u1 + ld);
             L.hs.pre_have = L.hs.abern && R.pre_it == it;
             L.hs.pre_offer = L.hs.xnext != nullptr;
+            L.hs.pre_head = ph;
         }
     }
     vk::Prelude& pr = L.pr;
@@ -456,6 +460,7 @@
     pr.sqrtMt = std::sqrt((double)c->Mt);
     pr.bern = R.bern;
     pr.bern_next = L.hs.xnext ? R.bern_next : nullptr;
+    pr.ahead = L.hs.abnext ? 1 : 0;
     pr.zero[0] = R.invQ;
     pr.zero[1] = L.rec ? R.tmpM : nullptr;
     L.pre_in_cg = R.fuse && (L.hs_av || L.arec);
@@ -540,7 +545,7 @@
         if (arec) HIPCHK(hipMemsetAsync(R.ax2, 0, (size_t)ld * 8, c->st));
     }
     const PreMode pm = R.pre_ahead == it ? PreMode::queued : PreMode::normal;
-    if (pm == PreMode::queued && !(L.pre_in_cg && R.fuse && hs_av))
+    if (pm == PreMode::queued && !(L.pre_in_cg && R.fuse && hs_av && pr.ahead == R.pre_ahead_look))
         return fail(VAMPOMI_ERR_STATE, "vamp: the start queued ahead does not match this iteration's schedule");
     if (!L.pre_in_cg) HIPCHK(vk::prelude(M, pr, c->st));
     const auto t_solve = std::chrono::steady_clock::now();
@@ -558,8 +563,14 @@
         pargs.hs = &hs;
         pargs.pre = &pr;
         pargs.pm = pm;
+        if (hs.abnext && R.hs2_it != it + 1) {
+            HIPCHK(vk::bernoulli(R.prm.seed, it + 1, c->S, M, pr.sqrtMt, so.d, c->st));
+            const double* xs[1] = {so.d};
+            STCHK(ax_dev(c, 1, xs, const_cast<double*>(hs.abnext)));
+        }
         STCHK(pcg_run(c, {&so, &sx}, pargs));
-        R.hs_it = hs.xnext ? it + 1 : 0;
+        R.hs_it = (hs.abnext || hs.xnext) ? it + 1 : 0;
+        R.hs2_it = hs.abnext ? it + 2 : 0;
         R.pre_it = hs.pre_made ? it + 1 : 0;
         c->pre_made_n += hs.pre_made ? 1 : 0;
         c->pre_used_n += hs.pre_used ? 1 : 0;
@@ -573,7 +584,7 @@
         }
         pargs.onepass = R.onepass;
         STCHK(pcg_run(c, {&sx, &so}, pargs));
-        R.hs_it = R.pre_it = 0;
+        R.hs_it = R.hs2_it = R.pre_it = 0;
     } else {
         R.pre_it = 0;
         PcgArgs first = pargs;
@@ -756,6 +767,7 @@
         pargs.pm = PreMode::ahead;
         STCHK(pcg_run(c, {&A.so, &A.sx}, pargs));
         R.pre_ahead = it + 1;
+        R.pre_ahead_look = A.pr.ahead;
     }
     STCHK(fin.flush());
     if (devem) {
```

Result: no change. 184.9, median of 6 (+0.6%).
